# engcang/FAST-LIO-SAM-QN

Measured on AMD Instinct MI355X. Metric: scan-pair registrations/sec on 100k-pt clouds, higher is better.
Workload: dtype f32 search / f64 accumulate

## Files before the change

### fast-lio-sam-qn_amd/csrc/qn_batch.inc

```

namespace {

template <class F> void lanes_launch(const void* tab, dim3 grid, hipStream_t s, uint32_t shmem) {
  hipLaunchKernelGGL(HIP_KERNEL_NAME(k_lanes<F>), grid, dim3(F::TB), shmem, s, (const LaneEntry<typename F::Args>*)tab);
}
template <class A> void lane_push(std::vector<LaneEntry<A>>& v, const A& a, uint32_t nbx) {
  LaneEntry<A> e; memset((void*)&e, 0, sizeof(e)); e.a = a; e.nbx = nbx; v.push_back(e);
}

struct LanePlan {
  qn_ctx* c; size_t off = 0; bool overflow = false; int flush_rc = QN_OK;
  struct Item { void (*fn)(const void*, dim3, hipStream_t, uint32_t); size_t off; dim3 grid; int family; uint32_t shmem; };
  std::vector<Item> items;
  explicit LanePlan(qn_ctx* c_) : c(c_) {}
  template <class F> void add(const std::vector<LaneEntry<typename F::Args>>& e, int family, uint32_t shmem = 0) {
    if (e.empty()) return;
    size_t a = (off + 255) & ~(size_t)255; const size_t bytes = sizeof(LaneEntry<typename F::Args>) * e.size();
    if (a + bytes > c->args_cap) {
      if (items.empty() || bytes > c->args_cap || flush_rc != QN_OK) { overflow = true; return; }
      flush_rc = run();
      if (flush_rc == QN_OK && hipStreamSynchronize(c->stream) != hipSuccess) { c->last_error = "batch: stream synchronisation failed while flushing the argument arena"; flush_rc = QN_ERR_HIP; }
      if (flush_rc != QN_OK) { overflow = true; return; }
      a = 0;
    }
    memcpy(c->args_h + a, e.data(), bytes);
    uint32_t gx = 0; for (const auto& x : e) gx = std::max(gx, x.nbx);
    gx = (gx + 7u) & ~7u;
    items.push_back(Item{&lanes_launch<F>, a, dim3(gx, (uint32_t)e.size()), family, shmem});
    off = a + bytes;
  }
  int run() {
    if (overflow) { if (flush_rc == QN_OK) c->last_error = "batch: argument arena too small for one launch's table"; return QN_ERR_HIP; }
    if (items.empty()) return QN_OK;
    HIPCHK(c, hipMemcpyAsync(c->args_d, c->args_h, off, hipMemcpyHostToDevice, c->stream));
    for (const Item& it : items) { c->prof_begin(it.family, (int)it.grid.y); it.fn(c->args_d + it.off, it.grid, c->stream, it.shmem); c->prof_end(); }
    c->batch_launches += items.size();
    items.clear(); off = 0;
    HIPCHK(c, hipGetLastError());
    return QN_OK;
  }
};

struct ScratchSwap {
  qn_ctx* c;
  static void sw(qn_ctx* c) {
    std::swap(c->scan_sums, c->scan_sums2); std::swap(c->fb_list, c->fb_list2); std::swap(c->big_list, c->big_list2); std::swap(c->fb_count2, c->fb_count2b);
    std::swap(c->knn_idx, c->knn_idx2); std::swap(c->bbox_acc, c->bbox_acc2); std::swap(c->scan_status, c->scan_status2); std::swap(c->staging, c->staging2); std::swap(c->pin_up, c->pin_up2);
  }
  explicit ScratchSwap(qn_ctx* c_) : c(c_) { sw(c); }
  ~ScratchSwap() { sw(c); }
};

struct LaneRun {
  qn_ctx* c = nullptr; uint32_t pair = 0; bool active = false;
  int alias = -1;
  int ticks_left = 0, chunk = 0, chunk_start = 0, next = 0; bool first_chunk = true; long budget = 0;
  bool build_source = true;
};

int lane_set_cloud(qn_ctx* c, int which, const float* xyz, uint32_t n, uint32_t stride, bool on_device, hipStream_t s, GridLaunch* out) {
  CloudBuf& b = c->cloud[which];
  b.n = 0; b.has_grid = b.has_cov = false;
  if (n == 0) return QN_ERR_EMPTY_CLOUD;
  if (!xyz || stride < 12 || (stride & 3)) return QN_ERR_INVALID_ARG;
  if (n > c->max_points) return QN_ERR_CAPACITY;
  const char* dsrc = (const char*)xyz;
  if (!on_device) { const int rc = upload_host_cloud(c, xyz, n, stride, s, &dsrc); if (rc != QN_OK) return rc; }
  b.n = n;
  *out = prep_grid(c, b, dsrc, stride, true);
  return QN_OK;
}

bool batch_supported(const qn_ctx* c) {
  const qn_gicp_params& p = c->params;
  const int maxit = p.force_iterations > 0 ? p.force_iterations : p.max_iterations;
  return c->batch_lanes >= 2 && !c->lanes_failed && maxit > 0 && c->fused_ticks && c->fused_final && c->far_enabled && c->knn_hist && !c->verify_track && !c->clk_probe && !c->list_probe &&
         c->tick_tb == 512 && c->tick_occ >= 4 && !c->dbg_counters;
}

int batch_ensure_lanes(qn_ctx* c) {
  HIPCHK(c, hipSetDevice(c->device));
  const int B = std::max(1, std::min(c->batch_lanes, 64));
  if (c->lanes.empty()) c->lanes.push_back(c);
  while ((int)c->lanes.size() < B) {
    qn_ctx* l = nullptr;
    const int rc = (c->fail_lane_create > 0 && (int)c->lanes.size() >= c->fail_lane_create) ? QN_ERR_HIP : ctx_create(c->device, c->max_points, c->stream, &l);
    if (rc != QN_OK) {
      c->last_error = "batch: lane context creation failed (lanes need batch_lanes x the context's device memory)";
      while (c->lanes.size() > 1) { qn_ctx_destroy(c->lanes.back()); c->lanes.pop_back(); }
      (void)hipGetLastError();
      c->lanes_failed = true;
      return rc;
    }
    c->lanes.push_back(l);
  }
  if (!c->args_h) {
    c->args_cap = (size_t)4 << 20;
    HIPCHK(c, hipHostMalloc(&c->args_h, c->args_cap, hipHostMallocDefault));
    HIPCHK(c, hipMalloc(&c->args_d, c->args_cap));
  }
  for (qn_ctx* l : c->lanes) {
    if (l == c) continue;
    if (l->params.k_correspondences != c->params.k_correspondences) l->cloud[0].has_cov = l->cloud[1].has_cov = false;
    l->params = c->params;
    l->cell_override = c->cell_override; l->margin_nn = c->margin_nn; l->margin_nn_t0 = c->margin_nn_t0; l->margin_knn = c->margin_knn; l->big_blocks0 = c->big_blocks0; l->fb_blocks0 = c->fb_blocks0;
    l->big_ratio = c->big_ratio; l->nn_rounds = c->nn_rounds; l->knn_rounds = c->knn_rounds; l->knn_trips = c->knn_trips; l->knn_mm = c->knn_mm; l->knn_single_all = c->knn_single_all; l->bbox_blocks = c->bbox_blocks; l->stable_cells = c->stable_cells;
    l->unseeded_cap = c->unseeded_cap; l->track_from_tick = c->track_from_tick; l->fused_from_tick = c->fused_from_tick; l->ticks_per_chunk = c->ticks_per_chunk; l->far_chunk = c->far_chunk; l->far_group = c->far_group; l->far_ranked = c->far_ranked;
    l->list_small = c->list_small; l->tick_ppt_min = c->tick_ppt_min; l->tick_rpb = c->tick_rpb; l->nn_lane = c->nn_lane;
  }
  return QN_OK;
}

int batch_register(qn_ctx* owner, const qn_pair_desc* pairs, const uint32_t* idx, uint32_t m, double thr, qn_gicp_result* results, int* valid, int* status,
                   std::vector<const float*>& last_src, std::vector<uint64_t>& last_key) {
  hipStream_t s = owner->stream;
  const auto t_call = std::chrono::steady_clock::now();
  const qn_gicp_params& p = owner->params;
  const int k = p.k_correspondences;
  LanePlan plan(owner);
  std::vector<LaneRun> L(m);
  struct AliasGuard {
    std::vector<LaneRun>& L; std::vector<CloudBuf> saved; std::vector<double*> saved_nrm; std::vector<const float*>& last_src;
    AliasGuard(std::vector<LaneRun>& L_, std::vector<const float*>& ls) : L(L_), saved(L_.size()), saved_nrm(L_.size(), nullptr), last_src(ls) {}
    void borrow(size_t l, qn_ctx* from) { qn_ctx* c = L[l].c; saved[l] = c->cloud[0]; saved_nrm[l] = c->nrm_s_sorted; c->cloud[0] = from->cloud[0]; c->nrm_s_sorted = from->nrm_s_sorted; }
    ~AliasGuard() { for (size_t l = 0; l < L.size(); l++) if (L[l].alias >= 0 && saved_nrm[l]) { qn_ctx* c = L[l].c; c->cloud[0] = saved[l]; c->nrm_s_sorted = saved_nrm[l]; c->cloud[0].has_grid = c->cloud[0].has_cov = false; c->cloud[0].n = 0; last_src[l] = nullptr; } }
  } alias_guard(L, last_src);
  struct FailGuard { std::vector<LaneRun>& L; int* status; bool armed = true; ~FailGuard() { if (armed) for (const LaneRun& R : L) if (R.active) status[R.pair] = QN_ERR_HIP; } } fail_guard{L, status};
  std::vector<LaneEntry<PackBBoxK::Args>> v_pack; std::vector<LaneEntry<CellCountK::Args>> v_count; std::vector<LaneEntry<ScanLookbackK::Args>> v_scan;
  std::vector<LaneEntry<ScatterK::Args>> v_scat; std::vector<LaneEntry<StableCellsK::Args>> v_stab;
  std::vector<LaneEntry<KnnHistArgs>> v_sel, v_lst; std::vector<LaneEntry<KnnSingleK::Args>> v_single; std::vector<LaneEntry<KnnCovArgs>> v_tail; std::vector<LaneEntry<CovFromIdxK::Args>> v_cov;
  auto push_grid = [&](const GridLaunch& G) {
    lane_push(v_pack, G.pack, G.pack_nb); lane_push(v_count, G.count, G.nb); lane_push(v_scan, G.scan, G.scan_nb); lane_push(v_scat, G.scat, G.nb);
    if (G.stable) lane_push(v_stab, G.stab, G.nb);
  };
  auto push_knn = [&](const KnnLaunch& K) {
    lane_push(v_sel, K.sel, K.sel_nb); lane_push(v_lst, K.lst, K.lst_nb); lane_push(v_single, K.single, K.single_nb); lane_push(v_tail, K.tail, K.tail_nb); lane_push(v_cov, K.cov, K.cov_nb);
  };
  for (uint32_t l = 0; l < m; l++) {
    LaneRun& R = L[l]; R.c = owner->lanes[l]; R.pair = idx[l];
    qn_ctx* c = R.c;
    const qn_pair_desc& pd = pairs[R.pair];
    qn_gicp_result* out = &results[R.pair];
    valid[R.pair] = 0; memset(out, 0, sizeof(*out)); out->fitness = DBL_MAX;
    for (int i = 0; i < 4; i++) { out->T[5 * i] = 1.f; out->T64[5 * i] = 1.0; }
    c->pair_pipeline = false; c->persist_batch_off = true; c->tgt_pending = false; c->tgt_on_stream2 = false;
    const uint64_t key = ((uint64_t)pd.ns << 32) ^ ((uint64_t)pd.stride_bytes << 1) ^ (uint64_t)(pd.on_device ? 1 : 0);
    R.build_source = !(owner->batch_share_source && last_src[l] == pd.src && last_key[l] == key && pd.src != nullptr && c->cloud[0].has_grid && c->cloud[0].has_cov && c->cloud[0].n == pd.ns);
    if (R.build_source && owner->batch_share_source && pd.src != nullptr && pd.ns > 0) {
      for (uint32_t j = 0; j < l; j++) {
        const qn_pair_desc& pj = pairs[L[j].pair];
        if (L[j].active && L[j].alias < 0 && pj.src == pd.src && pj.ns == pd.ns && pj.stride_bytes == pd.stride_bytes && pj.on_device == pd.on_device) { R.alias = (int)j; break; }
      }
      if (R.alias >= 0) { alias_guard.borrow(l, L[R.alias].c); R.build_source = false; }
    }
    int rc = QN_OK; GridLaunch gs, gt;
    if (R.build_source) { last_src[l] = nullptr; rc = lane_set_cloud(c, QN_SOURCE, pd.src, pd.ns, pd.stride_bytes, pd.on_device != 0, s, &gs); }
    if (rc == QN_OK) { ScratchSwap sw(c); rc = lane_set_cloud(c, QN_TARGET, pd.dst, pd.nt, pd.stride_bytes, pd.on_device != 0, s, &gt); }
    if (rc == QN_ERR_HIP) return rc;
    status[R.pair] = rc;
    if (rc != QN_OK) {
      if (R.build_source) { c->cloud[0].has_grid = c->cloud[0].has_cov = false; c->cloud[0].n = 0; }
      c->cloud[1].has_grid = c->cloud[1].has_cov = false; c->cloud[1].n = 0;
      continue;
    }
    if (R.build_source) { push_grid(gs); push_knn(prep_knn(c, c->cloud[0], k, c->knn_idx, nullptr, true)); c->cloud[0].has_cov = true; }
    { ScratchSwap sw(c); push_grid(gt); push_knn(prep_knn(c, c->cloud[1], k, c->knn_idx, nullptr, true)); c->cloud[1].has_cov = true; }
    last_src[l] = R.alias >= 0 ? nullptr : pd.src; last_key[l] = key;
    R.active = true;
  }
  plan.add<PackBBoxK>(v_pack, QN_K_GRID_BUILD); plan.add<CellCountK>(v_count, QN_K_GRID_BUILD); plan.add<ScanLookbackK>(v_scan, QN_K_GRID_BUILD); plan.add<ScatterK>(v_scat, QN_K_GRID_BUILD); plan.add<StableCellsK>(v_stab, QN_K_GRID_BUILD);
  if (k <= 24) { if (owner->knn_mm) plan.add<KnnHistK<false, 32>>(v_sel, QN_K_KNN_SELECT, (uint32_t)owner->knn_lds_pad); else plan.add<KnnHistK<false, 32, false>>(v_sel, QN_K_KNN_SELECT, (uint32_t)owner->knn_lds_pad); plan.add<KnnHistK<true, 32>>(v_lst, QN_K_KNN_COV); } else { plan.add<KnnHistK<false, 48>>(v_sel, QN_K_KNN_SELECT); plan.add<KnnHistK<true, 48>>(v_lst, QN_K_KNN_COV); }
  plan.add<KnnSingleK>(v_single, QN_K_KNN_COV);
  if (k <= 16) plan.add<KnnCovK<16, true, 4>>(v_tail, QN_K_KNN_COV); else if (k <= 20) plan.add<KnnCovK<20, true, 4>>(v_tail, QN_K_KNN_COV); else if (k <= 24) plan.add<KnnCovK<24, true, 4>>(v_tail, QN_K_KNN_COV); else plan.add<KnnCovK<32, true, 4>>(v_tail, QN_K_KNN_COV);
  plan.add<CovFromIdxK>(v_cov, QN_K_KNN_COV);

  const int per_outer = p.optimizer == QN_OPT_LM ? 2 : 1;
  const int maxit = p.force_iterations > 0 ? p.force_iterations : p.max_iterations;
  const int fixed_unseeded = std::max(1, std::min(owner->track_from_tick, owner->fused_from_tick)) * per_outer;
  const bool exact_ticks = p.force_iterations > 0 && p.optimizer == QN_OPT_GN;
  {
    std::vector<LaneEntry<InitStateK::Args>> v_init;
    for (LaneRun& R : L) {
      if (!R.active) continue;
      qn_ctx* c = R.c;
      c->gen = 0; c->part_rows = 0; c->far_mode = 2; c->clear_far_now = true; c->unseeded_until = fixed_unseeded; c->count_far_now = false;
      c->result_host->phase = 0;
      R.ticks_left = exact_ticks ? maxit : 1 << 30;
      R.chunk = std::min(fixed_unseeded, R.ticks_left); R.chunk_start = 0; R.next = R.chunk; R.first_chunk = true;
      R.budget = (long)maxit * (p.optimizer == QN_OPT_LM ? (p.lm_max_iterations + 1) : 1) + 2;
      lane_push(v_init, InitStateK::Args{st_cur(c), c->guess_tmp, 0, 0, c->far_stats}, 1u);
    }
    plan.add<InitStateK>(v_init, QN_K_SOLVE);
  }
  auto finish_lane = [&](LaneRun& R, int rc) {
    qn_ctx* c = R.c;
    R.active = false;
    status[R.pair] = rc;
    if (rc != QN_OK) return;
    results[R.pair] = c->result_host->r;
    c->trace_len = c->result_host->trace_len; c->aligned_valid = true;
    valid[R.pair] = (results[R.pair].converged && results[R.pair].fitness < thr) ? 1 : 0;
  };
  struct ProfFlush { qn_ctx* c; ~ProfFlush() { c->prof_collect(); } } prof_flush{owner};
  int tick_no = 0;
  for (;;) {
    int stop = 1 << 30; bool any = false;
    for (const LaneRun& R : L) if (R.active) { any = true; stop = std::min(stop, R.next); }
    if (!any) break;
    for (; tick_no < stop; tick_no++) {
      {
        std::vector<LaneEntry<NnSearchArgs>> v_g, v_l; std::vector<LaneEntry<AccumulateK::Args>> v_acc;
        bool group = true, lane = true;
        for (LaneRun& R : L) {
          if (!R.active || tick_no >= R.c->unseeded_until) continue;
          qn_ctx* c = R.c;
          const int t = tick_no - R.chunk_start;
          c->count_far_now = R.first_chunk && (t / per_outer == (R.chunk - 1) / per_outer);
          const NnLaunch N = prep_nn(c, 0, c->sqd, false, tick_no / per_outer, 0);
          group = group && N.group; lane = lane && N.lane;
          lane_push(v_g, N.grid, N.grid_nb); lane_push(v_l, N.list, N.list_nb);
          const uint32_t nb = acc_blocks(c);
          lane_push(v_acc, prep_accumulate(c, 0, true), nb);
          c->count_far_now = false;
        }
        if (lane) plan.add<NnLaneK<0>>(v_g, QN_K_NN_SEARCH); else plan.add<NnSearchK<0, false, QN_NN_BLOCK>>(v_g, QN_K_NN_SEARCH);
        if (group) plan.add<NnSearchK<0, true, QN_BLOCK, true>>(v_l, QN_K_NN_FALLBACK); else plan.add<NnSearchK<0, true, QN_BLOCK>>(v_l, QN_K_NN_FALLBACK);
        plan.add<AccumulateK>(v_acc, QN_K_ACCUMULATE);
      }
      {
        std::vector<LaneEntry<TickArgs>> v_t; std::vector<LaneEntry<FarArgs>> v_f; std::vector<LaneEntry<FarReduceK::Args>> v_r;
        for (LaneRun& R : L) {
          if (!R.active || tick_no < R.c->unseeded_until) continue;
          qn_ctx* c = R.c;
          const TickArgs a = tick_args(c);
          lane_push(v_t, a, tick_blocks(c));
          if (a.far_mode == 1) { lane_push(v_f, far_args(c), (uint32_t)QN_FAR_BLOCKS); lane_push(v_r, far_reduce_args(c), 1u); }
          c->gen++; c->part_rows = -1;
        }
        plan.add<TickK<512, 4, 0, false>>(v_t, QN_K_GN_TICK_FUSED, (uint32_t)owner->tick_lds_pad); plan.add<FarK>(v_f, QN_K_FAR); plan.add<FarReduceK>(v_r, QN_K_FAR);
      }
    }
    {
      std::vector<LaneEntry<FinalizeK::Args>> v_fin; std::vector<LaneEntry<TickArgs>> v_close; std::vector<LaneEntry<FinalizeFitK::Args>> v_fit;
      for (LaneRun& R : L) {
        if (!R.active || R.next != stop) continue;
        qn_ctx* c = R.c;
        if (exact_ticks && R.ticks_left > R.chunk) lane_push(v_fin, FinalizeK::Args{st_cur(c), c->result_host, c->far_stats}, 1u);
        else {
          const TickArgs a = tick_args(c, 1);
          const uint32_t nb = tick_blocks(c);
          lane_push(v_close, a, nb);
          lane_push(v_fit, FinalizeFitK::Args{st_cur(c), c->result_host, c->far_stats, c->fit_psum, c->fit_pcnt, (int)tick_rows(c)}, 1u);
        }
// ... 68 lines not shown
```

### fast-lio-sam-qn_amd/csrc/qn_context.h

```cpp
#pragma once
#include <hip/hip_runtime.h>
#include <string>
#include <vector>
#include "qn_gicp_kernels.cuh"

struct CloudBuf {
  uint32_t n = 0, ncells = 0;
  bool has_grid = false, has_cov = false;
  float4* raw = nullptr;
  float4* sorted = nullptr;
  float4* sorted_tmp = nullptr;
  uint32_t* cell_of_pt = nullptr;
  uint32_t* cell_start = nullptr;
  uint32_t* counts = nullptr;
  double* nrm = nullptr;
  qn::GridView grid{};
  qn::GridDims* dims = nullptr;
  qn::GridDims* dims_host = nullptr;
};

struct ProfSpan { int family; hipEvent_t a, b; int count; };

struct qn_ctx {
  int device = 0;
  uint32_t max_points = 0, max_cells = 0;
  hipStream_t stream = nullptr; bool owns_stream = true;
  std::vector<qn_ctx*> lanes; int batch_lanes = 8; char* args_h = nullptr; char* args_d = nullptr; size_t args_cap = 0; uint64_t batch_launches = 0, batch_pairs = 0; bool is_lane = false, batch_trace = false, batch_share_source = true;
  bool lanes_failed = false; int fail_lane_create = 0;
  void* slab = nullptr;
  qn_gicp_params params{};
  CloudBuf cloud[2];
  qn::BBoxAcc* bbox_acc = nullptr; qn::BBoxAcc* bbox_acc2 = nullptr;
  unsigned long long* scan_status = nullptr; unsigned long long* scan_status2 = nullptr; uint32_t build_epoch = 0;
  int far_group = -1;
  int far_chunk = 2;
  bool batch_look = false;
  bool far_ranked = true;
  unsigned long long* list_probe = nullptr;
  bool device_look = true;
  bool clear_far_now = false;
  char* staging2 = nullptr;
  struct PinZone { char* h = nullptr; hipEvent_t ev = nullptr; bool busy = false; } pin_up, pin_up2;
  char* staging = nullptr;
  uint32_t* scan_sums = nullptr;

  qn::GicpState* state = nullptr;
  uint32_t gen = 0; int part_rows = 0;
  double* partials = nullptr;
  uint32_t* tail_ticket = nullptr;
  double* fit_psum = nullptr; uint32_t* fit_pcnt = nullptr;
  qn_iter_trace* trace = nullptr; uint32_t trace_len = 0;
  int32_t* corr = nullptr; int32_t* nn_idx = nullptr; int32_t* knn_idx = nullptr; float4* nn_ref = nullptr; double* nrm_s_sorted = nullptr; qn::TargetRec* tgt_rec = nullptr; float* sqd = nullptr; float* sqd_fit = nullptr;
  int32_t* far_cand = nullptr; float4* far_cand_ref = nullptr; float2* far_cand_b = nullptr; unsigned long long* far_req = nullptr; uint32_t* far_stats = nullptr; double* far_rows = nullptr; int far_mode = 2; bool far_enabled = true;
  uint2* fb_list = nullptr; uint2* big_list = nullptr; uint32_t* fb_count2 = nullptr;
  float4* aligned = nullptr; bool aligned_valid = false;
  double* pose_tmp = nullptr; float* guess_tmp = nullptr;
  qn::ResultBlock* result_host = nullptr; double* scalar_host = nullptr;
  int32_t* dbg_knn_idx = nullptr; float* dbg_knn_d2 = nullptr;
  qn_quatro_params qparams{}; bool qparams_set = false, q_ready = false; double q_last_scale = 1.0;
  float4* q_normals[2] = {nullptr, nullptr}; float* q_spfh[2] = {nullptr, nullptr}; float* q_fpfh_s[2] = {nullptr, nullptr}; float* q_fpfh[2] = {nullptr, nullptr};
  unsigned long long* q_key[2] = {nullptr, nullptr};
  float* q_pair[2] = {nullptr, nullptr}; uint32_t* q_pair_hash[2] = {nullptr, nullptr};
  uint32_t* q_hit = nullptr; uint32_t* q_list = nullptr; uint32_t* q_sel = nullptr; uint2* q_pairs = nullptr; uint32_t* q_counts = nullptr; double* q_T = nullptr;
  void* q_mm_c = nullptr; void* q_mm_q = nullptr; float* q_mm_qn = nullptr; uint32_t* q_mm_L = nullptr; unsigned long long* q_mm_table = nullptr; unsigned long long* q_mm_table_q = nullptr; bool feat_query_dedupe = false;
  uint32_t q_mm_mask = 0;
  uint2* q_mm_pairs = nullptr; uint32_t* q_mm_cnt = nullptr; uint32_t q_mm_cap = 0, q_mm_ncnt = 0; bool feat_mfma = true, feat_mm_retry = false; int feat_sample = 4 ; bool feat_verify = false; int feat_min_blocks = 1536; double q_wall_ms[3] = {0, 0, 0}; unsigned long long* q_mm_vkeys = nullptr; uint32_t* q_mm_vcnt = nullptr; uint32_t feat_fallbacks = 0, feat_survivors = 0;
  bool c2f_overlap = false;
  bool c2f_lanes_fpfh = false;
  bool tgt_early = true;
  bool quatro_fused = true;
  int normals_fg = 0, fpfh_fg = 0;
  float4* c2f_src = nullptr; float4* c2f_dst = nullptr;
  float* q_mean = nullptr; double* q_mean_psum = nullptr; void* q_host = nullptr;
  double cell_override = 0.0;
  int list_small = 6000;
  float big_ratio = 2.5f;
  bool fused_ticks = true;
  int nn_rounds = 1;
  int nn_lane = -1;
  int track_from_tick = 3;
  int fused_from_tick = 3;
  int unseeded_until = 3; bool count_far_now = false; int last_extra_unseeded = 0;
  int unseeded_cap = 10;
  int single_from_tick = 2;
  bool fused_final = true;
  int knn_rounds = 2;
  int knn_mm = 1;
  int knn_trips = 3;
  int knn_hist = 1;
  int big_blocks0 = 4096, fb_blocks0 = 512;
  float margin_nn_t0 = 0.f;
  float margin_nn = 1.f, margin_knn = 0.f;
  int margin_nn_cap = 3, margin_knn_cap = 5, ticks_per_chunk = 8; bool knn_single_all = false, stable_cells = true; int bbox_blocks = 64;
  hipStream_t stream2 = nullptr; hipEvent_t ev_pair = nullptr; bool pair_pipeline = true, pair_failed = false, tgt_on_stream2 = false, tgt_pending = false, no_pipe = false;
  uint32_t* scan_sums2 = nullptr; uint2* fb_list2 = nullptr; uint2* big_list2 = nullptr; uint32_t* fb_count2b = nullptr; int32_t* knn_idx2 = nullptr;
  uint32_t tick_ppt_min = 1;
  uint32_t tick_rpb = 2;
  uint32_t tick_tb = 512;
  int batch_min_share = 4;
  int knn_lds_pad = 0;
  int tick_lds_pad = 0;
  int tick_occ = 4;
  unsigned long long* pg_rows = nullptr; unsigned long long* pg_bc = nullptr; unsigned long long* pg_fit = nullptr; uint32_t* pg_status = nullptr; uint32_t* pg_status_host = nullptr;
  unsigned long long* pg_clk = nullptr; uint32_t pg_epoch = 0; bool prof_persist = false, persist = true, persist_batch_off = false, persist_fits = true; int persist_resident_blocks = 0; uint32_t persist_launches = 0, persist_gave_up = 0; unsigned long long persist_timeout = 25000000ull;
  uint32_t* dbg_counters = nullptr;
  unsigned long long* clk_probe = nullptr; uint32_t clk_n = 0;
  bool verify_track = false; int32_t* v_corr = nullptr; int32_t* v_nn_idx = nullptr; float* v_sqd = nullptr; float4* v_nn_ref = nullptr; uint32_t* v_counters = nullptr;
  bool prof_on = false, prof_open = false; int prof_depth = 0;
  std::vector<ProfSpan> spans;
  qn_kernel_stat stats[QN_K_COUNT] = {};
  std::string last_error;

  void set_error(const char* what, hipError_t e, int line);
  void prof_begin(int family, int count = 1); void prof_end(); void prof_collect();
};
```

### fast-lio-sam-qn_amd/csrc/qn_device.cuh

```cuda
#pragma once
#include <hip/hip_runtime.h>
#include <stdint.h>

namespace qn {

#define QN_TX 8
#define QN_TY 4
#define QN_TZ 4
#define QN_TILE_CELLS 128

struct GridDims {
  float ox, oy, oz, cell, inv_cell, eps;
  int nx, ny, nz, ntx, nty, ntz;
  uint32_t n;
  uint32_t ncells, nonfinite, pad;
};
struct GridView {
  const float4* pts;
  const uint32_t* cell_start;
  uint32_t* dbg;
  float ox, oy, oz, cell, inv_cell, eps;
  int nx, ny, nz;
  int ntx, nty, ntz;
  uint32_t n;
  const GridDims* dims;
};
__device__ __forceinline__ int uni(int v) { return __builtin_amdgcn_readfirstlane(v); }
__device__ __forceinline__ uint32_t uni(uint32_t v) { return (uint32_t)__builtin_amdgcn_readfirstlane((int)v); }
__device__ __forceinline__ float uni(float v) { return __int_as_float(__builtin_amdgcn_readfirstlane(__float_as_int(v))); }
__device__ __forceinline__ double uni(double v) { union { double d; int i[2]; } u; u.d = v; u.i[0] = __builtin_amdgcn_readfirstlane(u.i[0]); u.i[1] = __builtin_amdgcn_readfirstlane(u.i[1]); return u.d; }
__device__ __forceinline__ GridView grid_resolve(GridView g) {
  const GridDims d = *g.dims;
  g.ox = uni(d.ox); g.oy = uni(d.oy); g.oz = uni(d.oz); g.cell = uni(d.cell); g.inv_cell = uni(d.inv_cell); g.eps = uni(d.eps);
  g.nx = uni(d.nx); g.ny = uni(d.ny); g.nz = uni(d.nz); g.ntx = uni(d.ntx); g.nty = uni(d.nty); g.ntz = uni(d.ntz); g.n = uni(d.n);
  return g;
}

template <class A> struct alignas(16) LaneEntry { A a; uint32_t nbx; uint32_t pad_[3]; };
template <class F>
__global__ void __launch_bounds__(F::TB, F::OCC) k_lanes(const LaneEntry<typename F::Args>* __restrict__ tab) {
  const LaneEntry<typename F::Args>* e = tab + blockIdx.y;
  const uint32_t nbx = e->nbx;
  if (blockIdx.x >= nbx) return;
  F::run(e->a, blockIdx.x, nbx);
}

#define QN_INF_KEY 0xFFFFFFFFFFFFFFFFull

__device__ __forceinline__ int clampi(int v, int lo, int hi) { return v < lo ? lo : (v > hi ? hi : v); }
__device__ __forceinline__ int cell_coord(float v, float o, float inv, int n) {
  return clampi((int)floorf((v - o) * inv), 0, n - 1);
}
__device__ __forceinline__ uint32_t cell_key(const GridView& g, int x, int y, int z) {
  const uint32_t tile = ((uint32_t)(z >> 2) * g.nty + (y >> 2)) * g.ntx + (x >> 3);
  return (tile << 7) | ((z & 3) << 5) | ((y & 3) << 3) | (x & 7);
}
__device__ __forceinline__ unsigned long long pack_key(float d2, uint32_t idx) {
  return ((unsigned long long)__float_as_uint(d2) << 32) | idx;
}
__device__ __forceinline__ float key_d2(unsigned long long k) { return __uint_as_float((uint32_t)(k >> 32)); }
__device__ __forceinline__ uint32_t key_idx(unsigned long long k) { return (uint32_t)k; }

typedef float qn_f2 __attribute__((ext_vector_type(2)));
__device__ __forceinline__ float sqdist(float qx, float qy, float qz, float px, float py, float pz) {
  const qn_f2 q = {qx, qy}, p = {px, py};
  const qn_f2 d = q - p;
  const qn_f2 d2 = d * d;
  const float dz = qz - pz;
  return (d2.x + d2.y) + dz * dz;
}

__device__ __forceinline__ int rfl(int v) { return __builtin_amdgcn_readfirstlane(v); }
__device__ __forceinline__ uint32_t rflu(uint32_t v) { return (uint32_t)__builtin_amdgcn_readfirstlane((int)v); }
__device__ __forceinline__ int rdlane(int v, int l) { return __builtin_amdgcn_readlane(v, l); }
__device__ __forceinline__ uint32_t rdlane(uint32_t v, int l) { return (uint32_t)__builtin_amdgcn_readlane((int)v, l); }
__device__ __forceinline__ float rdlane(float v, int l) { return __int_as_float(__builtin_amdgcn_readlane(__float_as_int(v), l)); }

#if defined(QN_INST_GROUP) && QN_INST_GROUP == 10
__device__ __forceinline__ int wave_min_i(int v) {
#pragma unroll
  for (int o = 32; o > 0; o >>= 1) { int t = __shfl_xor(v, o); v = t < v ? t : v; }
  return v;
}
__device__ __forceinline__ int wave_max_i(int v) {
#pragma unroll
  for (int o = 32; o > 0; o >>= 1) { int t = __shfl_xor(v, o); v = t > v ? t : v; }
  return v;
}
__device__ __forceinline__ unsigned long long wave_min_u64(unsigned long long v) {
#pragma unroll
  for (int o = 32; o > 0; o >>= 1) { unsigned long long t = __shfl_xor(v, o); v = t < v ? t : v; }
  return v;
}
__device__ __forceinline__ float wave_min_f(float v) {
#pragma unroll
  for (int o = 32; o > 0; o >>= 1) v = fminf(v, __shfl_xor(v, o));
  return v;
}
__device__ __forceinline__ float wave_max_f(float v) {
#pragma unroll
  for (int o = 32; o > 0; o >>= 1) v = fmaxf(v, __shfl_xor(v, o));
  return v;
}
// ... 166 lines not shown
  int k, cnt;
  __device__ __forceinline__ void reset() {
    w = QN_INF_KEY; cnt = 0;
    int kk = k; asm volatile("" : "+s"(kk));
#pragma unroll
    for (int j = 0; j < KMAX; j++) a[j] = (j < KMAX - kk) ? 0ull : QN_INF_KEY;
  }
  __device__ __forceinline__ void init(int k_, unsigned long long (*pend_)[64], uint32_t* dbg_ = nullptr) {
    k = k_; pend = pend_; dbg = dbg_; reset();
  }
  __device__ __forceinline__ bool slot_valid(int j) const { return j >= KMAX - k && a[j] != QN_INF_KEY; }
  __device__ __forceinline__ void refresh() { w = a[KMAX - 1]; }
  __device__ __forceinline__ void insert(unsigned long long key) {
#pragma unroll
    for (int j = 0; j < KMAX; j++) {
      unsigned long long lo = key < a[j] ? key : a[j];
      unsigned long long hi = key < a[j] ? a[j] : key;
      a[j] = lo; key = hi;
    }
  }
  __device__ __forceinline__ void flush() {
    const int lane = threadIdx.x & 63;
    const int m = wave_max_i(cnt);
    for (int e = 0; e < m; e++) {
      unsigned long long key = e < cnt ? pend[e][lane] : QN_INF_KEY;
      insert(key);
    }
    cnt = 0;
    refresh();
    if (dbg && lane == 0) atomicAdd(&dbg[2], 1u);
  }
  __device__ __forceinline__ void consider(bool on, float d2, uint32_t idx) {
    const unsigned long long key = pack_key(d2, idx);
    if (on && key < w) { pend[cnt][threadIdx.x & 63] = key; cnt++; }
    if (__any(cnt == QN_PEND_CAP)) flush();
  }
  __device__ __forceinline__ void merge_from(int lane_xor, bool recv) {
    if (KMAX > 24) {
      unsigned long long tmp[KMAX];
#pragma unroll
      for (int j = 0; j < KMAX; j++) tmp[j] = __shfl_xor(a[j], lane_xor);
#pragma unroll 1
      for (int j = 0; j < KMAX; j++) {
        unsigned long long other = QN_INF_KEY;
#pragma unroll
        for (int u = 0; u < KMAX; u++) other = (u == j) ? tmp[u] : other;
        if (__any(j >= KMAX - k)) insert((recv && j >= KMAX - k) ? other : QN_INF_KEY);
      }
      return;
    }
#pragma unroll
    for (int j = 0; j < KMAX; j++) {
      const unsigned long long other = __shfl_xor(a[j], lane_xor);
      if (__any(j >= KMAX - k)) insert((recv && j >= KMAX - k) ? other : QN_INF_KEY);
    }
  }
  template <int S>
  __device__ __forceinline__ void finish(bool on) {
    if (__any(cnt > 0)) flush();
    if (S == 1) return;
    const int lane = threadIdx.x & 63;
    merge_from(32, on && (lane & 32) == 0);
    if (S == 4) merge_from(16, on && (lane & 48) == 0);
    refresh();
    const unsigned long long w0 = __shfl(w, lane & (64 / S - 1));
    if (on) w = w0;
  }
  __device__ __forceinline__ bool full() const { return w != QN_INF_KEY; }
  __device__ __forceinline__ float worst_d2() const { return key_d2(w); }
  __device__ __forceinline__ int found() const {
    int f = 0;
#pragma unroll
    for (int j = 0; j < KMAX; j++) f += (j >= KMAX - k && a[j] != QN_INF_KEY) ? 1 : 0;
    return f;
  }
  __device__ __forceinline__ int wanted() const { return k; }
};

__device__ __forceinline__ float tile_box_d2(const GridView& g, int tx, int ty, int tz, float qx, float qy, float qz) {
  const float xl = g.ox + (float)(tx << 3) * g.cell, xh = g.ox + (float)min((tx << 3) + 8, g.nx) * g.cell;
  const float yl = g.oy + (float)(ty << 2) * g.cell, yh = g.oy + (float)min((ty << 2) + 4, g.ny) * g.cell;
  const float zl = g.oz + (float)(tz << 2) * g.cell, zh = g.oz + (float)min((tz << 2) + 4, g.nz) * g.cell;
  const float dx = fmaxf(fmaxf(xl - qx, qx - xh) - g.eps, 0.f), dy = fmaxf(fmaxf(yl - qy, qy - yh) - g.eps, 0.f), dz = fmaxf(fmaxf(zl - qz, qz - zh) - g.eps, 0.f);
  return ((dx * dx + dy * dy) + dz * dz) * 0.999998f;
}

__device__ __forceinline__ void divmod_small(int n, int d, int& q, int& r) {
  q = (int)((float)n * __builtin_amdgcn_rcpf((float)d));
  r = n - q * d;
  if (r < 0) { q--; r += d; }
  if (r >= d) { q++; r -= d; }
}

template <class Body>
__device__ __forceinline__ uint32_t stream_box(const GridView& g, int x0, int x1, int y0, int y1, int z0, int z1, const bool tile_mode, WaveLds* lds, Body&& body,
                                               const float bqx = 0.f, const float bqy = 0.f, const float bqz = 0.f, const float ball_r2 = -1.f) {
  const int lane = threadIdx.x & 63;
  const int tx0 = x0 >> 3, ntr = (x1 >> 3) - tx0 + 1, nyr = y1 - y0 + 1;
  const int ty0 = y0 >> 2, ntyr = (y1 >> 2) - ty0 + 1;
  const int nseg = tile_mode ? ntr * ntyr * ((z1 >> 2) - (z0 >> 2) + 1) : ntr * nyr * (z1 - z0 + 1);
  uint32_t grand = 0;
  for (int sb = 0; sb < nseg; sb += 64) {
    const int sidx = sb + lane;
    uint32_t s = 0, len = 0;
    if (sidx < nseg) {
      int t, r; divmod_small(sidx, ntr, r, t);
      if (tile_mode) {
        int qz_, ry_; divmod_small(r, ntyr, qz_, ry_);
        const int tzz = (z0 >> 2) + qz_, tyy = ty0 + ry_, txx = tx0 + t;
        const uint32_t tile = ((uint32_t)tzz * g.nty + tyy) * g.ntx + txx;
        if (!(ball_r2 >= 0.f && tile_box_d2(g, txx, tyy, tzz, bqx, bqy, bqz) > ball_r2)) { s = g.cell_start[tile << 7]; len = g.cell_start[(tile + 1) << 7] - s; }
      } else {
        int qz_, ry_; divmod_small(r, nyr, qz_, ry_);
        const int ry = y0 + ry_, rz = z0 + qz_, tx = tx0 + t;
        const int xa = max(x0, tx << 3), xb = min(x1, (tx << 3) + 7);
        const uint32_t k0 = cell_key(g, xa, ry, rz);
        s = g.cell_start[k0]; len = g.cell_start[k0 + (xb - xa) + 1] - s;
      }
    }
    const uint32_t incl = wave_incl_scan_u32(len, lane);
    const uint32_t total = rdlane(incl, 63);
    if (total == 0) continue;
    wave_lds_fence();
    lds->seg_excl[lane] = incl - len; lds->seg_start[lane] = s;
    wave_lds_fence();
    for (uint32_t cb = 0; cb < total; cb += 64) {
      const uint32_t slot = cb + lane;
      const bool valid = slot < total;
      const int j = chunk_segment(lds->tile_cid, cb, incl - len, incl);
      float4 p = make_float4(0.f, 0.f, 0.f, 0.f);
      if (valid) p = g.pts[lds->seg_start[j] + (slot - lds->seg_excl[j])];
      body(p, valid, min(64u, total - cb));
    }
    grand += total;
  }
  return grand;
}

#define QN_CL_DX 8
#define QN_CL_DY 4
#define QN_CL_DZ 4

template <int S>
__device__ __forceinline__ void build_clusters(const GridView& g, WaveLds* lds, unsigned long long todo, int cx, int cy, int cz,
                                               float qx, float qy, float qz, float r, uint32_t& cid, int& ncl, uint32_t& nseg_all) {
  const int lane = threadIdx.x & 63;
  const bool mine = (todo >> lane) & 1ull;
  cid = 0xffffffffu; ncl = 0;
  for (unsigned long long rem = todo; rem != 0; ncl++) {
    const int leader = __ffsll((long long)rem) - 1;
    const int ax = rdlane(cx, leader), ay = rdlane(cy, leader), az = rdlane(cz, leader);
    const bool in = ((rem >> lane) & 1ull) && abs(cx - ax) <= QN_CL_DX && abs(cy - ay) <= QN_CL_DY && abs(cz - az) <= QN_CL_DZ;
    if (in) cid = ncl;
    rem &= ~__ballot(in);
  }
  wave_lds_fence();
  if (lane < ncl) { lds->box[lane][0] = 0x3fffffff; lds->box[lane][1] = -1; lds->box[lane][2] = 0x3fffffff; lds->box[lane][3] = -1; lds->box[lane][4] = 0x3fffffff; lds->box[lane][5] = -1; }
  wave_lds_fence();
  if (mine && lane < 64 / S) {
    atomicMin(&lds->box[cid][0], cell_coord(qx - r, g.ox, g.inv_cell, g.nx)); atomicMax(&lds->box[cid][1], cell_coord(qx + r, g.ox, g.inv_cell, g.nx));
    atomicMin(&lds->box[cid][2], cell_coord(qy - r, g.oy, g.inv_cell, g.ny)); atomicMax(&lds->box[cid][3], cell_coord(qy + r, g.oy, g.inv_cell, g.ny));
    atomicMin(&lds->box[cid][4], cell_coord(qz - r, g.oz, g.inv_cell, g.nz)); atomicMax(&lds->box[cid][5], cell_coord(qz + r, g.oz, g.inv_cell, g.nz));
  }
  wave_lds_fence();
  uint32_t my_nseg = 0;
  if (lane < ncl) {
    int* b = lds->box[lane];
    my_nseg = (uint32_t)(((b[1] >> 3) - (b[0] >> 3) + 1) * (b[3] - b[2] + 1) * (b[5] - b[4] + 1));
    uint32_t tm = 0;
    if (my_nseg > 384) {
      tm = 1;
      b[0] = (b[0] >> 3) << 3; b[1] = min(((b[1] >> 3) << 3) + 7, g.nx - 1);
      b[2] = (b[2] >> 2) << 2; b[3] = min(((b[3] >> 2) << 2) + 3, g.ny - 1);
      b[4] = (b[4] >> 2) << 2; b[5] = min(((b[5] >> 2) << 2) + 3, g.nz - 1);
      my_nseg = (uint32_t)(((b[1] >> 3) - (b[0] >> 3) + 1) * ((b[3] >> 2) - (b[2] >> 2) + 1) * ((b[5] >> 2) - (b[4] >> 2) + 1));
    }
    lds->cl_tile_mode[lane] = tm;
  }
  const uint32_t seg_incl = wave_incl_scan_u32(my_nseg, lane);
  nseg_all = rdlane(seg_incl, 63);
  lds->cl_seg0[lane] = seg_incl - my_nseg;
  if (lane == 0) lds->cl_seg0[64] = nseg_all;
  wave_lds_fence();
}

template <int S, class Fn>
__device__ __forceinline__ void stream_chunks(const GridView& g, WaveLds* lds, const uint32_t total, Fn&& fn) {
  const int lane = threadIdx.x & 63;
  const float INF = __int_as_float(0x7f800000);
  const uint32_t ex = lds->seg_excl[lane], nxs = lane < 63 ? lds->seg_excl[(lane + 1) & 63] : total;
  for (uint32_t cb = 0; cb < total; cb += 64) {
    const uint32_t slot = cb + lane;
    const int j = chunk_segment(lds->tile_cid, cb, ex, nxs);
    const uint32_t cnt = min(64u, total - cb);
// ... 80 lines not shown
    bool retry = false;
    if (mine) {
      const int* b = lds->box[cid];
      const int ex0 = b[0], ex1 = b[1], ey0 = b[2], ey1 = b[3], ez0 = b[4], ez1 = b[5];
      const float INF = __int_as_float(0x7f800000);
      float d = INF;
      if (ex0 > 0) d = fminf(d, qx - (g.ox + ex0 * g.cell));
      if (ex1 < g.nx - 1) d = fminf(d, (g.ox + (ex1 + 1) * g.cell) - qx);
      if (ey0 > 0) d = fminf(d, qy - (g.oy + ey0 * g.cell));
      if (ey1 < g.ny - 1) d = fminf(d, (g.oy + (ey1 + 1) * g.cell) - qy);
      if (ez0 > 0) d = fminf(d, qz - (g.oz + ez0 * g.cell));
      if (ez1 < g.nz - 1) d = fminf(d, (g.oz + (ez1 + 1) * g.cell) - qz);
      if (d == INF || !(r == r)) { certified = true; d_unseen = INF; }
      else { d -= g.eps; d_unseen = d; certified = d > 0.f && sink.full() && sink.worst_d2() < d * d; }
      if (!certified) {
        if (sink.full()) r = fmaxf(sqrtf(sink.worst_d2()) * 1.000001f + g.eps, r + g.eps);
        else {
          const int f = sink.found();
          r = f > 0 ? fmaxf(r * sqrtf((float)sink.wanted() / (float)f) * 1.25f, r + g.cell) : 2.f * r + g.cell;
        }
        r = fminf(r, r_cap);
        if (round + 1 < max_rounds) { retry = true; sink.reset(); }
      }
    }
    todo = __ballot(retry);
    if (g.dbg && lane == 0 && todo) atomicAdd(&g.dbg[3], (uint32_t)__popcll(todo));
  }
  return certified;
}

struct CapBox {
  float o2[3];
  float S;
};
__device__ __forceinline__ CapBox cap_of(const GridView& g, float qx, float qy, float qz) {
  CapBox c;
  const float ox = fmaxf(fmaxf(g.ox - qx, qx - (g.ox + g.nx * g.cell)), 0.f);
  const float oy = fmaxf(fmaxf(g.oy - qy, qy - (g.oy + g.ny * g.cell)), 0.f);
  const float oz = fmaxf(fmaxf(g.oz - qz, qz - (g.oz + g.nz * g.cell)), 0.f);
  c.o2[0] = ox * ox; c.o2[1] = oy * oy; c.o2[2] = oz * oz; c.S = (c.o2[0] + c.o2[1]) + c.o2[2];
  return c;
}
__device__ __forceinline__ float cap_extent(const GridView& g, const CapBox& c, float r, int axis) {
  const float rest = c.S - c.o2[axis];
  if (rest <= 0.f) return r;
  const float v = r * r - rest * 0.999999f;
  return v > 0.f ? sqrtf(v) * 1.000001f + g.eps : g.eps;
}
__device__ __forceinline__ float cap_face_dist(const CapBox& c, float f, int axis) {
  const float rest = (c.S - c.o2[axis]) * 0.999999f;
  return rest > 0.f ? sqrtf(f * f + rest) * 0.999999f : f;
}

struct SingleStats { uint32_t rounds, cand, segs; float r_first, r_last; };
__device__ __forceinline__ void wave_search_single(const GridView& g, float qx, float qy, float qz, float r, const float r_cap,
                                                   unsigned long long& best_out, float& second_out, float& d_unseen, WaveLds* lds, SingleStats& st_out, const bool stats) {
  const int lane = threadIdx.x & 63;
  const float INF = __int_as_float(0x7f800000);
  const CapBox cap = cap_of(g, qx, qy, qz);
  if (cap.S > 0.f) r = fminf(fmaxf(r, sqrtf(cap.S) + g.cell), fmaxf(r_cap, r));
  if (stats) { st_out.rounds = 0; st_out.cand = 0; st_out.segs = 0; st_out.r_first = r; }
  float done2 = -1.f;
  int ptx0 = 0, ptx1 = -1, pty0 = 0, pty1 = -1, ptz0 = 0, ptz1 = -1;
  unsigned long long best = QN_INF_KEY; float second = INF;
  for (int round = 0;; round++) {
    const float rx = cap_extent(g, cap, r, 0), ry = cap_extent(g, cap, r, 1), rz = cap_extent(g, cap, r, 2);
    int x0 = rfl(cell_coord(qx - rx, g.ox, g.inv_cell, g.nx)), x1 = rfl(cell_coord(qx + rx, g.ox, g.inv_cell, g.nx));
    int y0 = rfl(cell_coord(qy - ry, g.oy, g.inv_cell, g.ny)), y1 = rfl(cell_coord(qy + ry, g.oy, g.inv_cell, g.ny));
    int z0 = rfl(cell_coord(qz - rz, g.oz, g.inv_cell, g.nz)), z1 = rfl(cell_coord(qz + rz, g.oz, g.inv_cell, g.nz));
    const int tx0 = x0 >> 3, ntr = (x1 >> 3) - tx0 + 1;
    int nseg = ntr * (y1 - y0 + 1) * (z1 - z0 + 1);
    const bool tile_mode = nseg > 128;
    int ty0 = 0, ntyr = 1;
    if (tile_mode) {
      x0 = (x0 >> 3) << 3; x1 = min(((x1 >> 3) << 3) + 7, g.nx - 1);
      y0 = (y0 >> 2) << 2; y1 = min(((y1 >> 2) << 2) + 3, g.ny - 1);
      z0 = (z0 >> 2) << 2; z1 = min(((z1 >> 2) << 2) + 3, g.nz - 1);
      ty0 = y0 >> 2; ntyr = (y1 >> 2) - ty0 + 1;
      nseg = ntr * ntyr * ((z1 >> 2) - (z0 >> 2) + 1);
    }
    const int nyr = y1 - y0 + 1;
    if (!tile_mode || done2 < 0.f) { best = QN_INF_KEY; second = INF; done2 = -1.f; }
    const float in2 = r * r * 1.000002f;
    for (int sb = 0; sb < nseg; sb += 64) {
      const int sidx = sb + lane;
      uint32_t s = 0, len = 0;
      if (sidx < nseg) {
        int t, rr; divmod_small(sidx, ntr, rr, t);
        if (tile_mode) {
          int qz_, ry_; divmod_small(rr, ntyr, qz_, ry_);
          const int tzz = (z0 >> 2) + qz_, tyy = ty0 + ry_, txx = tx0 + t;
          const uint32_t tile = ((uint32_t)tzz * g.nty + tyy) * g.ntx + txx;
          const float tb2 = tile_box_d2(g, txx, tyy, tzz, qx, qy, qz);
          const bool seen = tb2 <= done2 && txx >= ptx0 && txx <= ptx1 && tyy >= pty0 && tyy <= pty1 && tzz >= ptz0 && tzz <= ptz1;
          if (!(tb2 > in2) && !seen) { s = g.cell_start[tile << 7]; len = g.cell_start[(tile + 1) << 7] - s; }
        } else {
          int qz_, ry_; divmod_small(rr, nyr, qz_, ry_);
          const int ry = y0 + ry_, rz = z0 + qz_, tx = tx0 + t;
          const int xa = max(x0, tx << 3), xb = min(x1, (tx << 3) + 7);
          const uint32_t k0 = cell_key(g, xa, ry, rz);
          s = g.cell_start[k0]; len = g.cell_start[k0 + (xb - xa) + 1] - s;
        }
      }
      const uint32_t incl = wave_incl_scan_u32(len, lane);
      const uint32_t total = rdlane(incl, 63);
      if (total == 0) continue;
      if (g.dbg && lane == 0) atomicAdd(&g.dbg[11], total);
      if (stats) st_out.cand += total;
      wave_lds_fence();
      lds->seg_excl[lane] = incl - len; lds->seg_start[lane] = s;
      wave_lds_fence();
      for (uint32_t cb = 0; cb < total; cb += 64) {
        const uint32_t slot = cb + lane;
        const int j = chunk_segment(lds->tile_cid, cb, incl - len, incl);
        if (slot < total) {
          const float4 p = g.pts[lds->seg_start[j] + (slot - lds->seg_excl[j])];
          const float d2 = sqdist(qx, qy, qz, p.x, p.y, p.z);
          const unsigned long long k = pack_key(d2, __float_as_uint(p.w));
          if (k < best) { if (best != QN_INF_KEY) second = key_d2(best); best = k; }
          else if (d2 < second) second = d2;
        }
      }
    }
    if (g.dbg && lane == 0) { atomicAdd(&g.dbg[10], 1u); atomicAdd(&g.dbg[12], (uint32_t)nseg); if (round == 0) atomicAdd(&g.dbg[13], 1u); }
    if (stats) { st_out.rounds++; st_out.segs += (uint32_t)nseg; st_out.r_last = r; }
    if (tile_mode) { done2 = in2; ptx0 = tx0; ptx1 = tx0 + ntr - 1; pty0 = ty0; pty1 = ty0 + ntyr - 1; ptz0 = z0 >> 2; ptz1 = z1 >> 2; }
    const unsigned long long b = wave_min_u64(best);
    float c = (best == b) ? second : key_d2(best);
    if (best == QN_INF_KEY) c = INF;
    c = wave_min_f(c);
    float d = INF;
    if (x0 > 0) d = fminf(d, cap_face_dist(cap, qx - (g.ox + x0 * g.cell), 0));
    if (x1 < g.nx - 1) d = fminf(d, cap_face_dist(cap, (g.ox + (x1 + 1) * g.cell) - qx, 0));
    if (y0 > 0) d = fminf(d, cap_face_dist(cap, qy - (g.oy + y0 * g.cell), 1));
    if (y1 < g.ny - 1) d = fminf(d, cap_face_dist(cap, (g.oy + (y1 + 1) * g.cell) - qy, 1));
    if (z0 > 0) d = fminf(d, cap_face_dist(cap, qz - (g.oz + z0 * g.cell), 2));
    if (z1 < g.nz - 1) d = fminf(d, cap_face_dist(cap, (g.oz + (z1 + 1) * g.cell) - qz, 2));
    bool cert;
    if (tile_mode && r == r && round <= 160) d = fminf(d, r * 0.999998f + g.eps);
    if (d == INF || !(r == r) || round > 160) { cert = true; d_unseen = INF; }
    else { d -= g.eps; d_unseen = d; cert = d > 0.f && b != QN_INF_KEY && key_d2(b) < d * d; }
    if (cert) { best_out = b; second_out = c; return; }
    r = (b != QN_INF_KEY) ? fmaxf(sqrtf(key_d2(b)) * 1.000001f + g.eps, r + g.eps) : (r > 6.f * g.cell ? r + (2.f + round) * g.cell : 2.f * r + g.cell);
    r = fminf(r, r_cap);
  }
}

__device__ __forceinline__ void wave_search_single(const GridView& g, float qx, float qy, float qz, float r, const float r_cap,
                                                   unsigned long long& best_out, float& second_out, float& d_unseen, WaveLds* lds) {
  SingleStats none;
  wave_search_single(g, qx, qy, qz, r, r_cap, best_out, second_out, d_unseen, lds, none, false);
}

__device__ __forceinline__ void wave_search_far16(const GridView& g, float qx_in, float qy_in, float qz_in, bool member_in, float r_in,
                                                  unsigned long long& best_out, float& second_out, float& d_unseen_out, WaveLds* lds) {
  const int lane = threadIdx.x & 63;
  const float INF = __int_as_float(0x7f800000);
  const unsigned long long mm = __ballot(member_in) & 0xffffull;
  const int m = __popcll(mm);
  int m2 = 1; while (m2 < m) m2 <<= 1;
  const int S = 64 / m2;
  const int my_rank = __popcll(mm & ((1ull << (lane & 15)) - 1ull));
  wave_lds_fence();
  if (member_in && lane < 16) lds->seg_cid[my_rank] = (uint32_t)lane;
  wave_lds_fence();
  const int rk = lane & (m2 - 1);
  const bool has_q = rk < m;
  const int src_lane = has_q ? (int)lds->seg_cid[rk] : 0;
  const float qx = __shfl(qx_in, src_lane), qy = __shfl(qy_in, src_lane), qz = __shfl(qz_in, src_lane), r = __shfl(r_in, src_lane);
  const uint32_t sub = (uint32_t)(lane / m2);
  const float cqx = 0.5f * (wave_min_f(has_q ? qx : INF) + wave_max_f(has_q ? qx : -INF));
  const float cqy = 0.5f * (wave_min_f(has_q ? qy : INF) + wave_max_f(has_q ? qy : -INF));
  const float cqz = 0.5f * (wave_min_f(has_q ? qz : INF) + wave_max_f(has_q ? qz : -INF));
  const float off = has_q ? sqrtf(sqdist(qx, qy, qz, cqx, cqy, cqz)) * 1.000002f + 1e-30f : 0.f;
  float R = wave_max_f(has_q ? r + off : 0.f);
  const CapBox cap = cap_of(g, cqx, cqy, cqz);
  if (cap.S > 0.f) R = fmaxf(R, sqrtf(cap.S) + g.cell);
  Best1 sink; sink.init();
  bool open = has_q;
  unsigned long long fin_b = QN_INF_KEY; float fin_s = INF, fin_d = INF;
  float done2 = -1.f; int ptx0 = 0, ptx1 = -1, pty0 = 0, pty1 = -1, ptz0 = 0, ptz1 = -1;
  for (int round = 0;; round++) {
    const float rx = cap_extent(g, cap, R, 0), ry = cap_extent(g, cap, R, 1), rz = cap_extent(g, cap, R, 2);
    int x0 = rfl(cell_coord(cqx - rx, g.ox, g.inv_cell, g.nx)), x1 = rfl(cell_coord(cqx + rx, g.ox, g.inv_cell, g.nx));
    int y0 = rfl(cell_coord(cqy - ry, g.oy, g.inv_cell, g.ny)), y1 = rfl(cell_coord(cqy + ry, g.oy, g.inv_cell, g.ny));
    int z0 = rfl(cell_coord(cqz - rz, g.oz, g.inv_cell, g.nz)), z1 = rfl(cell_coord(cqz + rz, g.oz, g.inv_cell, g.nz));
    x0 = (x0 >> 3) << 3; x1 = min(((x1 >> 3) << 3) + 7, g.nx - 1);
    y0 = (y0 >> 2) << 2; y1 = min(((y1 >> 2) << 2) + 3, g.ny - 1);
    z0 = (z0 >> 2) << 2; z1 = min(((z1 >> 2) << 2) + 3, g.nz - 1);
    const int tx0 = x0 >> 3, ntr = (x1 >> 3) - tx0 + 1, ty0 = y0 >> 2, ntyr = (y1 >> 2) - ty0 + 1, tz0 = z0 >> 2;
    const int nseg = ntr * ntyr * ((z1 >> 2) - tz0 + 1);
    const float in2 = R * R * 1.000002f;
    bool left_out = false;
    for (int sb = 0; sb < nseg; sb += 64) {
      const int sidx = sb + lane;
      uint32_t s = 0, len = 0;
      if (sidx < nseg) {
        int t, rr; divmod_small(sidx, ntr, rr, t);
        int qz_, ry_; divmod_small(rr, ntyr, qz_, ry_);
        const int tzz = tz0 + qz_, tyy = ty0 + ry_, txx = tx0 + t;
        const uint32_t tile = ((uint32_t)tzz * g.nty + tyy) * g.ntx + txx;
        const float tb2 = tile_box_d2(g, txx, tyy, tzz, cqx, cqy, cqz);
        const bool seen = tb2 <= done2 && txx >= ptx0 && txx <= ptx1 && tyy >= pty0 && tyy <= pty1 && tzz >= ptz0 && tzz <= ptz1;
        if (tb2 > in2) left_out = true;
        else if (!seen) { s = g.cell_start[tile << 7]; len = g.cell_start[(tile + 1) << 7] - s; }
      }
      const uint32_t incl = wave_incl_scan_u32(len, lane);
      const uint32_t total = rdlane(incl, 63);
      if (total == 0) continue;
      if (g.dbg && lane == 0) atomicAdd(&g.dbg[11], total);
      wave_lds_fence();
      lds->seg_excl[lane] = incl - len; lds->seg_start[lane] = s;
      wave_lds_fence();
      for (uint32_t cb = 0; cb < total; cb += 64) {
        const uint32_t slot = cb + lane;
        const int j = chunk_segment(lds->tile_cid, cb, incl - len, incl);
        const uint32_t cnt = min(64u, total - cb);
        wave_lds_fence();
        if (slot < total) lds->tile[lane] = g.pts[lds->seg_start[j] + (slot - lds->seg_excl[j])];
        wave_lds_fence();
        for (uint32_t c = 0; c < cnt; c += 4u * (uint32_t)S) {
          float4 cp[4]; uint32_t ci[4];
#pragma unroll
          for (int u = 0; u < 4; u++) { ci[u] = c + (uint32_t)(u * S) + sub; cp[u] = lds->tile[ci[u] & 63u]; }
#pragma unroll
          for (int u = 0; u < 4; u++) sink.consider(open && ci[u] < cnt, sqdist(qx, qy, qz, cp[u].x, cp[u].y, cp[u].z), __float_as_uint(cp[u].w));
        }
      }
    }
    if (g.dbg && lane == 0) { atomicAdd(&g.dbg[10], 1u); atomicAdd(&g.dbg[12], (uint32_t)nseg); if (round == 0) atomicAdd(&g.dbg[13], 1u); }
    done2 = in2; ptx0 = tx0; ptx1 = tx0 + ntr - 1; pty0 = ty0; pty1 = ty0 + ntyr - 1; ptz0 = tz0; ptz1 = z1 >> 2;
    const bool everything = !__any(left_out) && x0 == 0 && x1 == g.nx - 1 && y0 == 0 && y1 == g.ny - 1 && z0 == 0 && z1 == g.nz - 1;
    unsigned long long b = sink.key;
    for (int o = m2; o < 64; o <<= 1) { const unsigned long long t = __shfl_xor(b, o); b = t < b ? t : b; }
    float sc = (sink.key == b) ? sink.second : key_d2(sink.key);
    if (sink.key == QN_INF_KEY) sc = INF;
    for (int o = m2; o < 64; o <<= 1) sc = fminf(sc, __shfl_xor(sc, o));
    float need = 0.f;
    if (open) {
      const float d = R * 0.999998f - off - g.eps;
      bool cert;
      if (everything || round > 160 || !(R == R)) { cert = true; fin_d = INF; }
      else { cert = d > 0.f && b != QN_INF_KEY && key_d2(b) < d * d; fin_d = fmaxf(d, 0.f); }
      if (cert) { fin_b = b; fin_s = sc; open = false; }
      else if (b != QN_INF_KEY) need = sqrtf(key_d2(b)) * 1.000002f + 2.f * g.eps + off;
    }
    if (!__any(open)) break;
    const float want = wave_max_f(need);
    const float grown = want > 0.f ? want : (R > 6.f * g.cell ? R + (2.f + round) * g.cell : 2.f * R + g.cell);
    R = fmaxf(grown, R * 1.0001f + g.eps);
  }
  const unsigned long long ob = __shfl(fin_b, my_rank & 63); const float os = __shfl(fin_s, my_rank & 63), od = __shfl(fin_d, my_rank & 63);
  if (member_in) { best_out = ob; second_out = os; d_unseen_out = od; }
}

template <int KMAX>
__device__ __forceinline__ void lane_ball_knn(const GridView& g, float qx, float qy, float qz, float r, BestK<KMAX>& sink) {
  for (int round = 0;; round++) {
    sink.reset();
    const int bx0 = cell_coord(qx - r, g.ox, g.inv_cell, g.nx), bx1 = cell_coord(qx + r, g.ox, g.inv_cell, g.nx);
    const int by0 = cell_coord(qy - r, g.oy, g.inv_cell, g.ny), by1 = cell_coord(qy + r, g.oy, g.inv_cell, g.ny);
    const int bz0 = cell_coord(qz - r, g.oz, g.inv_cell, g.nz), bz1 = cell_coord(qz + r, g.oz, g.inv_cell, g.nz);
    const bool all = bx0 == 0 && by0 == 0 && bz0 == 0 && bx1 == g.nx - 1 && by1 == g.ny - 1 && bz1 == g.nz - 1;
    for (int rz = bz0; rz <= bz1; rz++) for (int ry = by0; ry <= by1; ry++) for (int tx = bx0 >> 3; tx <= (bx1 >> 3); tx++) {
      const int xa = max(bx0, tx << 3), xb = min(bx1, (tx << 3) + 7);
      const uint32_t k0 = cell_key(g, xa, ry, rz);
      const uint32_t s = g.cell_start[k0], e = g.cell_start[k0 + (xb - xa) + 1];
      for (uint32_t i = s; i < e; i++) {
        const float4 p = g.pts[i];
        const unsigned long long key = pack_key(sqdist(qx, qy, qz, p.x, p.y, p.z), __float_as_uint(p.w));
        if (key < sink.w) { sink.insert(key); sink.refresh(); }
      }
    }
    if (all || round > 160) return;
    if (sink.full()) {
      const float bd = sqrtf(sink.worst_d2()) * 1.000001f + g.eps;
      if (bd <= r) return;
      r = bd;
    } else {
      r = 2.f * r + g.cell;
    }
  }
}

struct M3 { double m[3][3]; };

__device__ __forceinline__ M3 m3_inverse(const M3& a) {
  const double (*m)[3] = a.m;
  double c00 = m[1][1]*m[2][2] - m[1][2]*m[2][1];
  double c01 = m[1][2]*m[2][0] - m[1][0]*m[2][2];
  double c02 = m[1][0]*m[2][1] - m[1][1]*m[2][0];
  double det = m[0][0]*c00 + m[0][1]*c01 + m[0][2]*c02;
  double id = 1.0 / det;
  M3 r;
  r.m[0][0] = c00*id; r.m[1][0] = c01*id; r.m[2][0] = c02*id;
  r.m[0][1] = (m[0][2]*m[2][1] - m[0][1]*m[2][2])*id;
  r.m[1][1] = (m[0][0]*m[2][2] - m[0][2]*m[2][0])*id;
  r.m[2][1] = (m[0][1]*m[2][0] - m[0][0]*m[2][1])*id;
  r.m[0][2] = (m[0][1]*m[1][2] - m[0][2]*m[1][1])*id;
  r.m[1][2] = (m[0][2]*m[1][0] - m[0][0]*m[1][2])*id;
  r.m[2][2] = (m[0][0]*m[1][1] - m[0][1]*m[1][0])*id;
  return r;
}

__device__ inline void sym_eig3(const double A[6] , double w[3], double V[3][3]) {
  double a[3][3] = {{A[0], A[1], A[2]}, {A[1], A[3], A[4]}, {A[2], A[4], A[5]}};
  double v[3][3] = {{1, 0, 0}, {0, 1, 0}, {0, 0, 1}};
  for (int sweep = 0; sweep < 32; sweep++) {
    double off = fabs(a[0][1]) + fabs(a[0][2]) + fabs(a[1][2]);
    double diag = fabs(a[0][0]) + fabs(a[1][1]) + fabs(a[2][2]);
    if (off <= 1e-300 || off <= 1e-17 * diag) break;
#pragma unroll
    for (int pq = 0; pq < 3; pq++) {
      const int p = pq == 2 ? 1 : 0, q = pq == 0 ? 1 : 2;
      if (a[p][q] == 0.0) continue;
      double theta = (a[q][q] - a[p][p]) / (2.0 * a[p][q]);
      double t = (theta >= 0 ? 1.0 : -1.0) / (fabs(theta) + sqrt(theta * theta + 1.0));
      double c = 1.0 / sqrt(t * t + 1.0), s = t * c;
#pragma unroll
      for (int k = 0; k < 3; k++) { double akp = a[k][p], akq = a[k][q]; a[k][p] = c*akp - s*akq; a[k][q] = s*akp + c*akq; }
#pragma unroll
      for (int k = 0; k < 3; k++) { double apk = a[p][k], aqk = a[q][k]; a[p][k] = c*apk - s*aqk; a[q][k] = s*apk + c*aqk; }
#pragma unroll
      for (int k = 0; k < 3; k++) { double vkp = v[k][p], vkq = v[k][q]; v[k][p] = c*vkp - s*vkq; v[k][q] = s*vkp + c*vkq; }
    }
  }
  double e0 = a[0][0], e1 = a[1][1], e2 = a[2][2];
  int i0 = 0, i1 = 1, i2 = 2;
  if (e0 < e1) { double t = e0; e0 = e1; e1 = t; int ti = i0; i0 = i1; i1 = ti; }
  if (e1 < e2) { double t = e1; e1 = e2; e2 = t; int ti = i1; i1 = i2; i2 = ti; }
  if (e0 < e1) { double t = e0; e0 = e1; e1 = t; int ti = i0; i0 = i1; i1 = ti; }
  w[0] = e0; w[1] = e1; w[2] = e2;
// ... 10 lines not shown
```

### fast-lio-sam-qn_amd/csrc/qn_engine.hip

```cpp
#include <hip/hip_runtime.h>
#include <cfloat>
#include <cmath>
#include <cstdio>
#include <cstring>
#include <string>
#include <vector>
#include <atomic>
#include <thread>
#include <chrono>
#include "qn_instances.h"
#include "qn_context.h"
#include "qn_selftest.cuh"
#include "qn_pool.h"

using namespace qn;

#define HIPCHK(ctx, call)                                                                 \
  do { hipError_t e_ = (call);                                                            \
       if (e_ != hipSuccess) { (ctx)->set_error(#call, e_, __LINE__); return QN_ERR_HIP; } \
  } while (0)

void qn_ctx::set_error(const char* what, hipError_t e, int line) {
  char buf[512]; snprintf(buf, sizeof(buf), "%s -> %s (qn_engine.hip:%d)", what, hipGetErrorString(e), line);
  last_error = buf;
}

void qn_ctx::prof_begin(int family, int count) {
  if (!prof_on) return;
  if (prof_open) { prof_depth++; return; }
  ProfSpan sp; sp.family = family; sp.count = count;
  if (hipEventCreate(&sp.a) != hipSuccess) return;
  if (hipEventCreate(&sp.b) != hipSuccess) { hipEventDestroy(sp.a); return; }
  hipEventRecord(sp.a, stream);
  spans.push_back(sp);
  prof_open = true; prof_depth = 0;
}
void qn_ctx::prof_end() {
  if (!prof_on || spans.empty() || !prof_open) return;
  if (prof_depth > 0) { prof_depth--; return; }
  prof_open = false;
  hipEventRecord(spans.back().b, stream);
}
void qn_ctx::prof_collect() {
  for (auto& sp : spans) {
    float ms = 0; if (hipEventSynchronize(sp.b) == hipSuccess && hipEventElapsedTime(&ms, sp.a, sp.b) == hipSuccess) { stats[sp.family].total_ms += ms; stats[sp.family].launches += sp.count; }
    hipEventDestroy(sp.a); hipEventDestroy(sp.b);
  }
  spans.clear(); prof_open = false; prof_depth = 0;
}
struct ProfScope { qn_ctx* c; ProfScope(qn_ctx* c_, int fam) : c(c_) { c->prof_begin(fam); } ~ProfScope() { c->prof_end(); } };

extern "C" const char* qn_status_str(int s) {
  switch (s) {
    case QN_OK: return "ok"; case QN_ERR_INVALID_ARG: return "invalid argument"; case QN_ERR_EMPTY_CLOUD: return "empty cloud";
    case QN_ERR_CAPACITY: return "cloud exceeds context capacity"; case QN_ERR_NOT_READY: return "clouds/covariances not set";
    case QN_ERR_HIP: return "HIP runtime error"; case QN_ERR_NO_DEVICE: return "no gfx950 device (no CPU fallback)";
  }
  return "unknown status";
}
extern "C" const char* qn_last_error(const qn_ctx* ctx) { return ctx ? ctx->last_error.c_str() : "null context"; }

extern "C" void qn_gicp_default_params(qn_gicp_params* p) {
  if (!p) return;
  memset(p, 0, sizeof(*p));
  p->k_correspondences = 20; p->max_iterations = 64; p->max_corr_dist = (double)FLT_MAX;
  p->transformation_epsilon = 5e-4; p->rotation_epsilon = 2e-3; p->optimizer = QN_OPT_LM;
  p->lm_max_iterations = 10; p->lm_init_lambda_factor = 1e-9; p->force_iterations = 0;
  p->ransac_iterations = 0; p->ransac_outlier_threshold = 0.05; p->euclidean_fitness_epsilon = -DBL_MAX;
}

struct Slab {
  char* base = nullptr; size_t off = 0, cap = 0;
  template <class T> void take(T*& p, size_t bytes) {
    const size_t a = (off + 255) & ~(size_t)255;
    if (base) p = (T*)(base + a);
    off = a + bytes;
  }
};
static void carve_cloud(qn_ctx* c, Slab& sl, CloudBuf& b) {
  sl.take(b.raw, sizeof(float4) * c->max_points);
  sl.take(b.sorted, sizeof(float4) * c->max_points);
  sl.take(b.sorted_tmp, sizeof(float4) * c->max_points);
  sl.take(b.cell_of_pt, sizeof(uint32_t) * c->max_points);
  sl.take(b.cell_start, sizeof(uint32_t) * ((size_t)c->max_cells + 1));
  sl.take(b.counts, sizeof(uint32_t) * ((size_t)c->max_cells + 1));
  sl.take(b.nrm, sizeof(double) * 3 * c->max_points);
  sl.take(b.dims, sizeof(GridDims));
}

static int ctx_create(int device, uint32_t max_points, hipStream_t shared_stream, qn_ctx** out);
extern "C" int qn_ctx_create(int device, uint32_t max_points, qn_ctx** out) { return ctx_create(device, max_points, nullptr, out); }
static int ctx_create(int device, uint32_t max_points, hipStream_t shared_stream, qn_ctx** out) {
  if (!out || max_points == 0) return QN_ERR_INVALID_ARG;
  *out = nullptr;
  int ndev = 0;
  if (hipGetDeviceCount(&ndev) != hipSuccess || ndev <= 0 || device < 0 || device >= ndev) return QN_ERR_NO_DEVICE;
  qn_ctx* c = new qn_ctx();
  c->device = device; c->max_points = max_points;
  size_t mc = (size_t)max_points * 16; if (mc < (1u << 18)) mc = 1u << 18; if (mc > (1u << 23)) mc = 1u << 23;
  c->max_cells = (uint32_t)mc;
  qn_gicp_default_params(&c->params);
  int rc = QN_OK;
  auto fail = [&](int code) { qn_ctx_destroy(c); return code; };
  if (hipSetDevice(device) != hipSuccess) return fail(QN_ERR_NO_DEVICE);
  if (shared_stream) { c->stream = shared_stream; c->owns_stream = false; c->is_lane = true; }
  else if (hipStreamCreateWithFlags(&c->stream, hipStreamNonBlocking) != hipSuccess) return fail(QN_ERR_HIP);
#define CA(call) if ((call) != hipSuccess) return fail(QN_ERR_HIP)
  auto carve = [&](Slab& sl) {
    carve_cloud(c, sl, c->cloud[0]);
    carve_cloud(c, sl, c->cloud[1]);
    sl.take(c->staging, (size_t)max_points * 32);
    sl.take(c->scan_sums, sizeof(uint32_t) * (c->max_cells / (QN_BLOCK * QN_SCAN_ITEMS) + 2));
    sl.take(c->state, 2 * sizeof(GicpState));
    sl.take(c->partials, 2 * sizeof(double) * (QN_ACC_MAX_BLOCKS + 8) * QN_NPART);
    sl.take(c->nn_idx, sizeof(int32_t) * max_points);
    sl.take(c->knn_idx, sizeof(int32_t) * (size_t)max_points * 32);
    sl.take(c->nn_ref, sizeof(float4) * max_points);
    sl.take(c->nrm_s_sorted, sizeof(double) * 3 * max_points);
    sl.take(c->tgt_rec, sizeof(TargetRec) * max_points);
    sl.take(c->fit_psum, sizeof(double) * (QN_ACC_MAX_BLOCKS + 8));
    sl.take(c->fit_pcnt, sizeof(uint32_t) * (QN_ACC_MAX_BLOCKS + 8));
    sl.take(c->trace, sizeof(qn_iter_trace) * QN_MAX_TRACE);
    sl.take(c->corr, sizeof(int32_t) * max_points);
    sl.take(c->sqd, sizeof(float) * max_points);
    sl.take(c->sqd_fit, sizeof(float) * max_points);
    sl.take(c->far_cand, sizeof(int32_t) * QN_FAR_M * (size_t)max_points);
    sl.take(c->far_cand_ref, sizeof(float4) * max_points);
    sl.take(c->far_cand_b, sizeof(float2) * max_points);
    sl.take(c->far_req, sizeof(unsigned long long) * (max_points / 64 + 2));
    sl.take(c->far_stats, 4 * sizeof(uint32_t));
    sl.take(c->far_rows, sizeof(double) * QN_FAR_BLOCKS * QN_NPART);
    sl.take(c->fb_list, sizeof(uint2) * max_points);
    sl.take(c->big_list, sizeof(uint2) * max_points);
    sl.take(c->fb_count2, 4 * sizeof(uint32_t));
    sl.take(c->aligned, sizeof(float4) * max_points);
    sl.take(c->pose_tmp, sizeof(double) * 16);
    sl.take(c->guess_tmp, sizeof(float) * 16);
    sl.take(c->scan_sums2, sizeof(uint32_t) * (c->max_cells / (QN_BLOCK * QN_SCAN_ITEMS) + 2));
    sl.take(c->fb_list2, sizeof(uint2) * max_points);
    sl.take(c->big_list2, sizeof(uint2) * max_points);
    sl.take(c->fb_count2b, 4 * sizeof(uint32_t));
    sl.take(c->knn_idx2, sizeof(int32_t) * (size_t)max_points * 32);
    sl.take(c->staging2, (size_t)max_points * 32);
    sl.take(c->bbox_acc, 2 * (QN_BBOX_MAX_BLOCKS + 1) * sizeof(BBoxAcc)); c->bbox_acc2 = c->bbox_acc ? c->bbox_acc + (QN_BBOX_MAX_BLOCKS + 1) : nullptr;
    sl.take(c->scan_status, sizeof(unsigned long long) * 2 * (c->max_cells / (QN_BLOCK * QN_SCAN_ITEMS) + 2)); c->scan_status2 = c->scan_status ? c->scan_status + (c->max_cells / (QN_BLOCK * QN_SCAN_ITEMS) + 2) : nullptr;
    sl.take(c->pg_rows, sizeof(unsigned long long) * 3 * QN_PERSIST_ROWS * QN_PERSIST_RSTRIDE);
    sl.take(c->pg_bc, sizeof(unsigned long long) * 64);
    sl.take(c->pg_fit, sizeof(unsigned long long) * (QN_PERSIST_MAX_BLOCKS + 1) * 4);
    sl.take(c->pg_status, 4 * sizeof(uint32_t));
    sl.take(c->tail_ticket, 4 * sizeof(uint32_t));
  };
  { Slab dry; carve(dry);
    Slab sl; sl.cap = (dry.off + ((size_t)2 << 20) - 1) & ~(((size_t)2 << 20) - 1);
    CA(hipMalloc(&c->slab, sl.cap)); sl.base = (char*)c->slab; carve(sl); }
  CA(hipMemsetAsync(c->far_stats, 0, 4 * sizeof(uint32_t), c->stream));
  CA(hipHostMalloc(&c->result_host, sizeof(ResultBlock), hipHostMallocDefault));
  for (int w = 0; w < 2; w++) { CA(hipHostMalloc(&c->cloud[w].dims_host, sizeof(GridDims), hipHostMallocDefault)); memset(c->cloud[w].dims_host, 0, sizeof(GridDims)); }
  CA(hipHostMalloc(&c->scalar_host, 64 * sizeof(double), hipHostMallocDefault));
  CA(hipHostMalloc(&c->pg_status_host, 4 * sizeof(uint32_t), hipHostMallocDefault));
  CA(hipMemsetAsync(c->pg_rows, 0xFF, sizeof(unsigned long long) * 3 * QN_PERSIST_ROWS * QN_PERSIST_RSTRIDE, c->stream));
  CA(hipMemsetAsync(c->pg_bc, 0, sizeof(unsigned long long) * 64, c->stream));
  CA(hipMemsetAsync(c->pg_fit, 0, sizeof(unsigned long long) * (QN_PERSIST_MAX_BLOCKS + 1) * 4, c->stream));
  CA(hipMemsetAsync(c->pg_status, 0, 4 * sizeof(uint32_t), c->stream));
  CA(hipMemsetAsync(c->tail_ticket, 0, 4 * sizeof(uint32_t), c->stream));
  CA(hipMemsetAsync(c->state, 0, 2 * sizeof(GicpState), c->stream));
  hipLaunchKernelGGL(k_bbox_acc_init, dim3(1), dim3(256), 0, c->stream, c->bbox_acc, 2 * (QN_BBOX_MAX_BLOCKS + 1));
  CA(hipMemsetAsync(c->fb_count2, 0, 4 * sizeof(uint32_t), c->stream)); CA(hipMemsetAsync(c->fb_count2b, 0, 4 * sizeof(uint32_t), c->stream));
  CA(hipMemsetAsync(c->scan_status, 0, sizeof(unsigned long long) * 2 * (c->max_cells / (QN_BLOCK * QN_SCAN_ITEMS) + 2), c->stream));
  for (int w = 0; w < 2; w++) CA(hipMemsetAsync(c->cloud[w].counts, 0, sizeof(uint32_t) * ((size_t)c->max_cells + 1), c->stream));
  CA(hipMemsetAsync(c->knn_idx, 0xff, sizeof(int32_t) * (size_t)max_points * 32, c->stream));
// ... 18 lines not shown
  for (qn_ctx* l : c->lanes) if (l != c) qn_ctx_destroy(l);
  c->lanes.clear();
  if (c->args_h) hipHostFree(c->args_h);
  hipFree(c->args_d);
  c->prof_collect();
  hipFree(c->slab);
  hipFree(c->q_mm_c); hipFree(c->q_mm_q); hipFree(c->q_mm_qn); hipFree(c->q_mm_L); hipFree(c->q_mm_table); hipFree(c->q_mm_table_q); hipFree(c->q_mm_pairs); hipFree(c->q_mm_cnt); hipFree(c->q_mm_vkeys); hipFree(c->q_mm_vcnt);
  for (int w = 0; w < 2; w++) { hipFree(c->q_normals[w]); hipFree(c->q_spfh[w]); hipFree(c->q_fpfh_s[w]); hipFree(c->q_fpfh[w]); hipFree(c->q_key[w]); hipFree(c->q_pair[w]); hipFree(c->q_pair_hash[w]); }
  hipFree(c->q_hit); hipFree(c->q_list); hipFree(c->q_sel); hipFree(c->q_pairs); hipFree(c->q_counts); hipFree(c->q_T); hipFree(c->q_mean); hipFree(c->q_mean_psum);
  if (c->q_host) hipHostFree(c->q_host);
  hipFree(c->c2f_src); hipFree(c->c2f_dst);
  hipFree(c->dbg_knn_idx); hipFree(c->dbg_knn_d2); hipFree(c->dbg_counters);
  hipFree(c->v_corr); hipFree(c->v_nn_idx); hipFree(c->v_sqd); hipFree(c->v_nn_ref); hipFree(c->v_counters);
  if (c->result_host) hipHostFree(c->result_host);
  for (int w = 0; w < 2; w++) if (c->cloud[w].dims_host) hipHostFree(c->cloud[w].dims_host);
  if (c->scalar_host) hipHostFree(c->scalar_host);
  hipFree(c->pg_clk); if (c->list_probe) hipFree(c->list_probe); if (c->pg_status_host) hipHostFree(c->pg_status_host);
  if (c->ev_pair) hipEventDestroy(c->ev_pair);
  for (qn_ctx::PinZone* z : {&c->pin_up, &c->pin_up2}) { if (z->ev) hipEventDestroy(z->ev); if (z->h) hipHostFree(z->h); }
  if (c->stream2) { hipStreamSynchronize(c->stream2); hipStreamDestroy(c->stream2); }
  if (c->stream && c->owns_stream) hipStreamDestroy(c->stream);
  delete c;
}

static int clouds_valid(qn_ctx* c);
extern "C" void* qn_ctx_stream(qn_ctx* c) { return c ? (void*)c->stream : nullptr; }
extern "C" int qn_ctx_synchronize(qn_ctx* c) {
  if (!c) return QN_ERR_INVALID_ARG;
  HIPCHK(c, hipStreamSynchronize(c->stream));
  if (c->stream2) HIPCHK(c, hipStreamSynchronize(c->stream2));
  c->prof_collect();
  return clouds_valid(c);
}

extern "C" int qn_gicp_set_params(qn_ctx* c, const qn_gicp_params* p) {
  if (!c || !p) return QN_ERR_INVALID_ARG;
  if (p->k_correspondences < 1 || p->k_correspondences > 32 || p->max_iterations < 0 || p->lm_max_iterations < 1 ||
      (p->optimizer != QN_OPT_LM && p->optimizer != QN_OPT_GN) || !(p->max_corr_dist > 0)) return QN_ERR_INVALID_ARG;
  if (p->k_correspondences != c->params.k_correspondences) { c->cloud[0].has_cov = c->cloud[1].has_cov = false; }
  c->params = *p;
  return QN_OK;
}

extern "C" int qn_gicp_get_params(const qn_ctx* c, qn_gicp_params* p) { if (!c || !p) return QN_ERR_INVALID_ARG; *p = c->params; return QN_OK; }

static GicpConfig make_cfg(const qn_ctx* c) {
  GicpConfig g; const qn_gicp_params& p = c->params;
  g.k = p.k_correspondences; g.max_iterations = p.max_iterations; g.optimizer = p.optimizer; g.lm_max_iterations = p.lm_max_iterations;
  g.force_iterations = p.force_iterations; g.max_corr_dist_sq = p.max_corr_dist * p.max_corr_dist;
  g.transformation_epsilon = p.transformation_epsilon; g.rotation_epsilon = p.rotation_epsilon; g.lm_init_lambda_factor = p.lm_init_lambda_factor;
  return g;
}

static inline GicpState* st_cur(qn_ctx* c) { return c->state + (c->gen & 1u); }
static inline GicpState* st_nxt(qn_ctx* c) { return c->state + ((c->gen + 1u) & 1u); }
static inline double* part_cur(qn_ctx* c) { return c->partials + (size_t)(c->gen & 1u) * (QN_ACC_MAX_BLOCKS + 8) * QN_NPART; }
static inline double* part_nxt(qn_ctx* c) { return c->partials + (size_t)((c->gen + 1u) & 1u) * (QN_ACC_MAX_BLOCKS + 8) * QN_NPART; }

static bool pair_pipeline_ready(qn_ctx* c) {
  if (c->stream2) return true;
  if (c->pair_failed || !c->knn_idx2) return false;
  const bool ok = hipStreamCreateWithFlags(&c->stream2, hipStreamNonBlocking) == hipSuccess && hipEventCreateWithFlags(&c->ev_pair, hipEventDisableTiming) == hipSuccess;
  if (!ok) { c->pair_failed = true; if (c->stream2) { hipStreamDestroy(c->stream2); c->stream2 = nullptr; } (void)hipGetLastError(); }
  return ok;
}
static void swap_scratch(qn_ctx* c) {
  std::swap(c->stream, c->stream2); std::swap(c->scan_sums, c->scan_sums2); std::swap(c->fb_list, c->fb_list2); std::swap(c->big_list, c->big_list2);
  std::swap(c->fb_count2, c->fb_count2b); std::swap(c->knn_idx, c->knn_idx2);
  std::swap(c->bbox_acc, c->bbox_acc2); std::swap(c->scan_status, c->scan_status2);
  std::swap(c->pin_up, c->pin_up2);
  std::swap(c->staging, c->staging2);
}
struct TargetScope {
  qn_ctx* c; bool on;
  TargetScope(qn_ctx* c_, bool on_) : c(c_), on(on_) { if (on) swap_scratch(c); }
  ~TargetScope() { if (on) { (void)hipEventRecord(c->ev_pair, c->stream); swap_scratch(c); c->tgt_pending = true; } }
};
static int join_target(qn_ctx* c) {
  if (!c->tgt_pending) return QN_OK;
  c->tgt_pending = false;
  return hipStreamWaitEvent(c->stream, c->ev_pair, 0) == hipSuccess ? QN_OK : QN_ERR_HIP;
}

struct GridLaunch { PackBBoxK::Args pack; uint32_t pack_nb; CellCountK::Args count; ScanLookbackK::Args scan; uint32_t scan_nb; ScatterK::Args scat; StableCellsK::Args stab; bool stable; uint32_t nb; };
static GridLaunch prep_grid(qn_ctx* c, CloudBuf& b, const char* dsrc, uint32_t stride, bool lanes = false) {
  const uint32_t n = b.n;
  GridView& g = b.grid;
  memset(&g, 0, sizeof(g));
  g.pts = b.sorted; g.cell_start = b.cell_start; g.dbg = c->dbg_counters; g.n = n; g.dims = b.dims;
  GridLaunch L;
  L.nb = (n + QN_BLOCK - 1) / QN_BLOCK;
  L.scan_nb = (c->max_cells + QN_BLOCK * QN_SCAN_ITEMS - 1) / (QN_BLOCK * QN_SCAN_ITEMS);
  if (((++c->build_epoch) & 0x3fffffffu) == 0u) ++c->build_epoch;
  L.pack_nb = std::min<uint32_t>(L.nb, (uint32_t)std::min(lanes ? QN_BBOX_MAX_BLOCKS : c->bbox_blocks, QN_BBOX_MAX_BLOCKS));
  L.pack = PackBBoxK::Args{dsrc, stride, n, b.raw, c->bbox_acc, c->max_cells, c->cell_override, b.dims, b.dims_host};
  L.count = CellCountK::Args{b.raw, n, g, b.counts, b.cell_of_pt};
  L.scan = ScanLookbackK::Args{b.counts, b.dims, b.cell_start, c->scan_status, c->build_epoch, n};
  L.stable = c->stable_cells;
  L.scat = ScatterK::Args{b.raw, n, b.cell_of_pt, b.cell_start, b.counts, L.stable ? b.sorted_tmp : b.sorted};
  L.stab = StableCellsK::Args{b.sorted_tmp, n, b.cell_of_pt, b.cell_start, b.sorted};
  b.has_grid = true; b.has_cov = false;
  return L;
}
static int build_grid(qn_ctx* c, CloudBuf& b, const char* dsrc, uint32_t stride) {
  hipStream_t s = c->stream;
  const GridLaunch L = prep_grid(c, b, dsrc, stride);
  { ProfScope ps(c, QN_K_GRID_BUILD);
    hipLaunchKernelGGL(k_pack_bbox_dims, dim3(L.pack_nb), dim3(QN_BLOCK), 0, s, L.pack.in, L.pack.stride, L.pack.n, L.pack.raw, L.pack.acc, L.pack.max_cells, L.pack.cell_override, L.pack.dims_dev, L.pack.dims_host);
    hipLaunchKernelGGL(k_cell_count, dim3(L.nb), dim3(QN_BLOCK), 0, s, L.count.pts, L.count.n, L.count.g, L.count.counts, L.count.cell_of_pt);
    hipLaunchKernelGGL(k_scan_lookback, dim3(L.scan_nb), dim3(QN_BLOCK), 0, s, L.scan.in, L.scan.dims, L.scan.out, L.scan.status, L.scan.epoch, L.scan.total);
    hipLaunchKernelGGL(k_scatter, dim3(L.nb), dim3(QN_BLOCK), 0, s, L.scat.pts, L.scat.n, L.scat.cell_of_pt, L.scat.cell_start, L.scat.counts, L.scat.sorted);
    if (L.stable) hipLaunchKernelGGL(k_stable_cells, dim3(L.nb), dim3(QN_BLOCK), 0, s, L.stab.in, L.stab.n, L.stab.cell_of_pt, L.stab.cell_start, L.stab.out); }
  HIPCHK(c, hipGetLastError());
  return QN_OK;
}
static int clouds_valid(qn_ctx* c) {
  for (int w = 0; w < 2; w++)
    if (c->cloud[w].has_grid && c->cloud[w].dims_host && c->cloud[w].dims_host->nonfinite) {
      c->last_error = w == 0 ? "source cloud contains non-finite coordinates (is_dense == false clouds are not supported)" : "target cloud contains non-finite coordinates (is_dense == false clouds are not supported)";
      c->cloud[w].has_grid = c->cloud[w].has_cov = false;
      return QN_ERR_INVALID_ARG;
    }
  return QN_OK;
}

static int upload_host_cloud(qn_ctx* c, const float* xyz, uint32_t n, uint32_t& stride, hipStream_t s, const char** dsrc) {
  hipPointerAttribute_t at;
  const bool pinned = hipPointerGetAttributes(&at, xyz) == hipSuccess && at.type == hipMemoryTypeHost;
  if (!pinned) (void)hipGetLastError();
  if (pinned) {
    if (stride <= 32) { HIPCHK(c, hipMemcpyAsync(c->staging, xyz, (size_t)(n - 1) * stride + 12, hipMemcpyHostToDevice, s)); }
    else { HIPCHK(c, hipMemcpy2DAsync(c->staging, 16, xyz, stride, 16, n, hipMemcpyHostToDevice, s)); stride = 16; }
    *dsrc = (const char*)c->staging;
    return QN_OK;
  }
  qn_ctx::PinZone& z = c->pin_up;
  if (!z.h) { HIPCHK(c, hipHostMalloc((void**)&z.h, (size_t)c->max_points * 16, hipHostMallocDefault)); HIPCHK(c, hipEventCreateWithFlags(&z.ev, hipEventDisableTiming)); }
  if (z.busy) { HIPCHK(c, hipEventSynchronize(z.ev)); z.busy = false; }
  float* o = (float*)z.h; const char* in = (const char*)xyz;
  for (uint32_t i = 0; i < n; i++, in += stride, o += 3) { const float* p = (const float*)in; o[0] = p[0]; o[1] = p[1]; o[2] = p[2]; }
  HIPCHK(c, hipMemcpyAsync(c->staging, z.h, (size_t)n * 12, hipMemcpyHostToDevice, s));
  HIPCHK(c, hipEventRecord(z.ev, s)); z.busy = true;
  stride = 12; *dsrc = (const char*)c->staging;
  return QN_OK;
}

static int set_cloud(qn_ctx* c, int which, const float* xyz, uint32_t n, uint32_t stride, bool on_device) {
  if (!c || (which != 0 && which != 1)) return QN_ERR_INVALID_ARG;
  CloudBuf& b = c->cloud[which];
  b.n = 0; b.has_grid = b.has_cov = false;
  if (n == 0) return QN_ERR_EMPTY_CLOUD;
  if (!xyz || stride < 12 || (stride & 3)) return QN_ERR_INVALID_ARG;
  if (n > c->max_points) return QN_ERR_CAPACITY;
  HIPCHK(c, hipSetDevice(c->device));
  if (which == QN_SOURCE && join_target(c) != QN_OK) return QN_ERR_HIP;
  c->tgt_on_stream2 = which == QN_TARGET ? (c->pair_pipeline && !c->prof_on && !c->no_pipe && c->cloud[0].has_grid && pair_pipeline_ready(c)) : c->tgt_on_stream2;
  TargetScope scope(c, which == QN_TARGET && c->tgt_on_stream2);
  hipStream_t s = c->stream;
  const char* dsrc = (const char*)xyz;
  if (!on_device) { const int rc = upload_host_cloud(c, xyz, n, stride, s, &dsrc); if (rc != QN_OK) return rc; }
  b.n = n;
  return build_grid(c, b, dsrc, stride);
}

extern "C" int qn_gicp_set_source(qn_ctx* c, const float* xyz, uint32_t n, uint32_t stride) { return set_cloud(c, QN_SOURCE, xyz, n, stride, false); }
extern "C" int qn_gicp_set_target(qn_ctx* c, const float* xyz, uint32_t n, uint32_t stride) { return set_cloud(c, QN_TARGET, xyz, n, stride, false); }
extern "C" int qn_gicp_set_source_device(qn_ctx* c, const float* xyz, uint32_t n, uint32_t stride) { return set_cloud(c, QN_SOURCE, xyz, n, stride, true); }
extern "C" int qn_gicp_set_target_device(qn_ctx* c, const float* xyz, uint32_t n, uint32_t stride) { return set_cloud(c, QN_TARGET, xyz, n, stride, true); }

struct KnnLaunch { KnnHistArgs sel; uint32_t sel_nb; KnnHistArgs lst; uint32_t lst_nb; KnnSingleK::Args single; uint32_t single_nb; KnnCovArgs tail; uint32_t tail_nb; CovFromIdxK::Args cov; uint32_t cov_nb; };
static float knn_first_radius(const qn_ctx* c, const CloudBuf& b) {
  return -(c->margin_knn > 0.f ? c->margin_knn : (b.n > 16384u && b.n <= 65536u ? 2.5f : 2.0f));
}
static KnnLaunch prep_knn(qn_ctx* c, CloudBuf& b, int k, int32_t* kidx, float* kd2, bool lanes = false) {
  const float r0 = knn_first_radius(c, b);
  uint32_t* genc = c->fb_count2 + 1;
  KnnLaunch L;
  L.sel_nb = (b.n + QN_KNN_BLOCK / 4 - 1) / (QN_KNN_BLOCK / 4);
  if (lanes && c->knn_trips > 1) L.sel_nb = (L.sel_nb + (uint32_t)c->knn_trips - 1) / (uint32_t)c->knn_trips;
  L.sel = KnnHistArgs{b.grid, k, r0, c->knn_single_all ? -1 : c->knn_rounds, kidx, kd2, c->fb_list, c->fb_count2, c->big_list, genc};
  L.lst_nb = std::min<uint32_t>((b.n + 63) / 64, lanes ? 96 : 512) * (QN_BLOCK / QN_KNN_BLOCK);
  L.lst = KnnHistArgs{b.grid, k, r0, 64, kidx, kd2, c->fb_list, c->fb_count2, c->big_list, genc};
  L.single_nb = std::min<uint32_t>((b.n + 3) / 4, lanes ? 128 : 2048);
  L.single = KnnSingleK::Args{b.grid, k, kidx, kd2, c->big_list, genc, c->fb_list, c->fb_count2 + 2};
  L.tail_nb = std::min<uint32_t>((b.n + 63) / 64, lanes ? 64 : 1024);
  L.tail = KnnCovArgs{b.grid, b.raw, k, r0, 64, b.nrm, kidx, kd2, c->fb_list, c->fb_count2 + 2};
  L.cov_nb = (b.n + QN_BLOCK - 1) / QN_BLOCK;
  L.cov = CovFromIdxK::Args{b.raw, b.sorted, b.n, k, kidx, b.nrm, &b == &c->cloud[0] ? c->nrm_s_sorted : (double*)nullptr, &b == &c->cloud[0] ? (TargetRec*)nullptr : c->tgt_rec, c->fb_count2};
  return L;
}
template <int KMAX>
static void launch_knn_cov(qn_ctx* c, CloudBuf& b, int k, int32_t* kidx, float* kd2) {
  hipStream_t s = c->stream;
  if (c->knn_hist) {
    const KnnLaunch L = prep_knn(c, b, k, kidx, kd2);
// ... 606 lines not shown
  if (!T || !H || !b6 || !err) return QN_ERR_INVALID_ARG;
  HIPCHK(c, hipSetDevice(c->device));
  hipStream_t s = c->stream;
  HIPCHK(c, hipMemcpyAsync(c->pose_tmp, T, sizeof(double) * 16, hipMemcpyHostToDevice, s));
  hipLaunchKernelGGL(k_set_pose, dim3(1), dim3(64), 0, s, st_cur(c), c->pose_tmp, 0, 0);
  enqueue_nn(c, 0, c->sqd, false); enqueue_accumulate(c, 0, false); enqueue_solve(c, 1, 0);
  GicpState* hs = (GicpState*)malloc(sizeof(GicpState));
  hipError_t e = hipMemcpyAsync(hs, st_cur(c), sizeof(GicpState), hipMemcpyDeviceToHost, s);
  if (e == hipSuccess && corr_out) e = hipMemcpyAsync(corr_out, c->corr, sizeof(int32_t) * c->cloud[0].n, hipMemcpyDeviceToHost, s);
  if (e == hipSuccess && sqd_out) e = hipMemcpyAsync(sqd_out, c->sqd, sizeof(float) * c->cloud[0].n, hipMemcpyDeviceToHost, s);
  if (e == hipSuccess) e = hipStreamSynchronize(s);
  if (e != hipSuccess) { free(hs); c->set_error("linearize readback", e, __LINE__); return QN_ERR_HIP; }
  memcpy(H, hs->H, sizeof(double) * 36); memcpy(b6, hs->b, sizeof(double) * 6); *err = hs->y0;
  free(hs);
  c->prof_collect();
  return clouds_valid(c);
}

extern "C" int qn_gicp_compute_error(qn_ctx* c, const double T[16], double* err) {
  if (c && join_target(c) != QN_OK) return QN_ERR_HIP;
  int rc = ready(c); if (rc != QN_OK) return rc;
  if (!T || !err) return QN_ERR_INVALID_ARG;
  HIPCHK(c, hipSetDevice(c->device));
  hipStream_t s = c->stream;
  HIPCHK(c, hipMemcpyAsync(c->pose_tmp, T, sizeof(double) * 16, hipMemcpyHostToDevice, s));
  hipLaunchKernelGGL(k_set_pose, dim3(1), dim3(64), 0, s, st_cur(c), c->pose_tmp, 1, 1);
  enqueue_accumulate(c, 0, false); enqueue_solve(c, 2, 0);
  HIPCHK(c, hipMemcpyAsync(c->scalar_host, &st_cur(c)->yi, sizeof(double), hipMemcpyDeviceToHost, s));
  HIPCHK(c, hipStreamSynchronize(s));
  *err = c->scalar_host[0];
  c->prof_collect();
  return clouds_valid(c);
}

extern "C" int qn_prof_enable(qn_ctx* c, int on) { if (!c) return QN_ERR_INVALID_ARG; c->prof_on = on != 0; return QN_OK; }
extern "C" int qn_prof_reset(qn_ctx* c) { if (!c) return QN_ERR_INVALID_ARG; c->prof_collect(); for (auto& s : c->stats) { s.total_ms = 0; s.launches = 0; } return QN_OK; }
extern "C" int qn_prof_get(qn_ctx* c, int fam, qn_kernel_stat* out) {
  if (!c || !out || fam < 0 || fam >= QN_K_COUNT) return QN_ERR_INVALID_ARG;
  c->prof_collect(); *out = c->stats[fam]; return QN_OK;
}
extern "C" int qn_debug_set(qn_ctx* c, const char* key, double v) {
  if (!c || !key) return QN_ERR_INVALID_ARG;
  std::string k(key);
  if (k == "cell") { c->cell_override = v; c->cloud[0].has_grid = c->cloud[1].has_grid = false; }
  else if (k == "margin_nn") c->margin_nn = (float)v;
  else if (k == "margin_nn_t0") c->margin_nn_t0 = (float)v;
  else if (k == "big_blocks0") c->big_blocks0 = v < 64 ? 64 : (int)v;
  else if (k == "fb_blocks0") c->fb_blocks0 = v < 64 ? 64 : (int)v;
  else if (k == "margin_knn") c->margin_knn = (float)v;
  else if (k == "knn_single_all") c->knn_single_all = v != 0;
  else if (k == "bbox_blocks") c->bbox_blocks = std::max(1, (int)v);
  else if (k == "device_look") c->device_look = v != 0;
  else if (k == "far_group") c->far_group = (int)v;
  else if (k == "c2f_overlap") c->c2f_overlap = v != 0;
  else if (k == "quatro_fused") c->quatro_fused = v != 0;
  else if (k == "tgt_early") c->tgt_early = v != 0;
  else if (k == "c2f_lanes_fpfh") c->c2f_lanes_fpfh = v != 0;
  else if (k == "normals_fg") c->normals_fg = (int)v;
  else if (k == "fpfh_fg") c->fpfh_fg = (int)v;
  else if (k == "list_small") c->list_small = std::max(0, (int)v);
  else if (k == "far_chunk") c->far_chunk = std::max(1, (int)v);
  else if (k == "far_ranked") c->far_ranked = v != 0;
  else if (k == "batch_look") c->batch_look = v != 0;
  else if (k == "unseeded_cap") c->unseeded_cap = (int)v;
  else if (k == "pair_pipeline") c->pair_pipeline = v != 0;
  else if (k == "persist") c->persist = v != 0;
  else if (k == "persist_timeout") c->persist_timeout = v < 1 ? 1ull : (unsigned long long)v;
  else if (k == "prof_persist") c->prof_persist = v != 0;
  else if (k == "persist_probe") {
    if (v != 0 && !c->pg_clk) { if (hipMalloc(&c->pg_clk, 8 * (64 * 16 + 16)) != hipSuccess) return QN_ERR_HIP; }
    if (c->pg_clk) (void)hipMemset(c->pg_clk, 0, 8 * (64 * 16 + 16));
    if (v == 0) { (void)hipFree(c->pg_clk); c->pg_clk = nullptr; }
  }
  else if (k == "batch_lanes") {
    const int b = std::max(1, std::min((int)v, 64));
    if (b < (int)c->lanes.size()) { if (hipStreamSynchronize(c->stream) != hipSuccess) return QN_ERR_HIP; while ((int)c->lanes.size() > std::max(b, 1)) { qn_ctx* l = c->lanes.back(); c->lanes.pop_back(); if (l != c) qn_ctx_destroy(l); } }
    c->batch_lanes = b; c->lanes_failed = false;
  }
  else if (k == "fail_lane_create") c->fail_lane_create = (int)v;
  else if (k == "batch_share_source") c->batch_share_source = v != 0;
  else if (k == "batch_trace") c->batch_trace = v != 0;
  else if (k == "batch_member") c->persist_batch_off = v != 0;
  else if (k == "stable_cells") c->stable_cells = v != 0;
  else if (k == "knn_hist") c->knn_hist = v != 0;
  else if (k == "nn_rounds") c->nn_rounds = v < 1 ? 1 : (int)v;
  else if (k == "nn_lane") c->nn_lane = v < 0 ? -1 : (v != 0 ? 1 : 0);
  else if (k == "track_from_tick") c->track_from_tick = v < 1 ? 1 : (int)v;
  else if (k == "single_from_tick") c->single_from_tick = v < 1 ? 1 : (int)v;
  else if (k == "fused_from_tick") c->fused_from_tick = v < 1 ? 1 : (int)v;
  else if (k == "knn_rounds") c->knn_rounds = v < 1 ? 1 : (int)v;
  else if (k == "knn_trips") c->knn_trips = v < 1 ? 1 : (int)v;
  else if (k == "knn_mm") c->knn_mm = v != 0;
  else if (k == "fused_ticks") c->fused_ticks = v != 0;
  else if (k == "big_ratio") c->big_ratio = (float)v;
  else if (k == "margin_nn_cap") c->margin_nn_cap = (int)v;
  else if (k == "margin_knn_cap") c->margin_knn_cap = (int)v;
  else if (k == "dbg_counters") {
    if (v != 0 && !c->dbg_counters) { if (hipMalloc(&c->dbg_counters, 16 * sizeof(uint32_t)) != hipSuccess) return QN_ERR_HIP; }
    if (c->dbg_counters) (void)hipMemset(c->dbg_counters, 0, 16 * sizeof(uint32_t));
    if (v == 0) { (void)hipFree(c->dbg_counters); c->dbg_counters = nullptr; }
    for (int w = 0; w < 2; w++) c->cloud[w].grid.dbg = c->dbg_counters;
  }
  else if (k == "ticks_per_chunk") c->ticks_per_chunk = std::max(1, (int)v);
  else if (k == "tick_occ") c->tick_occ = (int)v;
  else if (k == "far") c->far_enabled = v != 0;
  else if (k == "fused_final") c->fused_final = v != 0;
  else if (k == "feat_mfma") c->feat_mfma = v != 0;
  else if (k == "feat_sample") c->feat_sample = (int)v;
  else if (k == "feat_query_dedupe") c->feat_query_dedupe = v != 0;
  else if (k == "feat_min_blocks") c->feat_min_blocks = (int)v;
  else if (k == "feat_verify") { c->feat_verify = v != 0; if (c->q_mm_vcnt) (void)hipMemset(c->q_mm_vcnt, 0, 16); }
  else if (k == "list_probe") {
    if (v != 0 && !c->list_probe) { if (hipMalloc(&c->list_probe, sizeof(unsigned long long) * 4 * 16384) != hipSuccess) return QN_ERR_HIP; }
    if (v == 0 && c->list_probe) { (void)hipFree(c->list_probe); c->list_probe = nullptr; }
  }
  else if (k == "clk_probe") {
    if (v != 0 && !c->clk_probe) { if (hipMalloc(&c->clk_probe, 8 * 8 * 256 + 8 * 12 * 1024) != hipSuccess) return QN_ERR_HIP; }
    if (c->clk_probe) (void)hipMemset(c->clk_probe, 0, 8 * 8 * 256 + 8 * 12 * 1024);
    c->clk_n = 0; if (v == 0) { (void)hipFree(c->clk_probe); c->clk_probe = nullptr; }
  }
  else if (k == "tick_tb") c->tick_tb = v >= 512 ? 512 : 256;
  else if (k == "tick_ppt_min") c->tick_ppt_min = v < 1 ? 1u : (uint32_t)v;
  else if (k == "tick_rpb") c->tick_rpb = v < 1 ? 1u : (uint32_t)v;
  else if (k == "tick_lds_pad") c->tick_lds_pad = v < 0 ? 0 : (int)v;
  else if (k == "knn_lds_pad") c->knn_lds_pad = v < 0 ? 0 : (int)v;
  else if (k == "batch_min_share") c->batch_min_share = v < 1 ? 1 : (int)v;
  else if (k == "verify_track") {
    if (v != 0 && !c->v_counters) {
      const size_t n = c->max_points;
      if (hipMalloc(&c->v_corr, 4 * n) != hipSuccess || hipMalloc(&c->v_nn_idx, 4 * n) != hipSuccess || hipMalloc(&c->v_sqd, 4 * n) != hipSuccess ||
          hipMalloc(&c->v_nn_ref, 16 * n) != hipSuccess || hipMalloc(&c->v_counters, 16) != hipSuccess) return QN_ERR_HIP;
    }
    if (c->v_counters) (void)hipMemset(c->v_counters, 0, 16);
    c->verify_track = v != 0;
  }
  else return QN_ERR_INVALID_ARG;
  return QN_OK;
}
extern "C" int qn_debug_selftest(qn_ctx* c, uint32_t n_waves, uint32_t seed, uint32_t* mismatches) {
  if (!c || !mismatches || n_waves == 0 || n_waves > 65536) return QN_ERR_INVALID_ARG;
  HIPCHK(c, hipSetDevice(c->device));
  std::vector<uint32_t> h((size_t)n_waves * 128);
  uint64_t x = 0x9e3779b97f4a7c15ull ^ seed;
  for (auto& v : h) { x ^= x << 13; x ^= x >> 7; x ^= x << 17; v = (uint32_t)(x >> 16); }
  uint32_t* d = nullptr;
  HIPCHK(c, hipMalloc(&d, (h.size() + 1) * sizeof(uint32_t)));
  int rc = QN_OK; uint32_t bad = 0xffffffffu;
  if (hipMemcpyAsync(d, h.data(), h.size() * sizeof(uint32_t), hipMemcpyHostToDevice, c->stream) != hipSuccess || hipMemsetAsync(d + h.size(), 0, sizeof(uint32_t), c->stream) != hipSuccess) rc = QN_ERR_HIP;
  if (rc == QN_OK) {
    hipLaunchKernelGGL(k_selftest_wave, dim3(n_waves), dim3(64), 0, c->stream, d, d + (size_t)n_waves * 64, d + h.size());
    if (hipMemcpyAsync(&bad, d + h.size(), sizeof(uint32_t), hipMemcpyDeviceToHost, c->stream) != hipSuccess || hipStreamSynchronize(c->stream) != hipSuccess) rc = QN_ERR_HIP;
  }
  (void)hipFree(d);
  if (rc != QN_OK) { c->last_error = "selftest: HIP call failed"; return rc; }
  *mismatches = bad;
  return QN_OK;
}
extern "C" int qn_debug_get_counters(qn_ctx* c, uint32_t out[16]) {
  if (!c || !c->dbg_counters) return QN_ERR_INVALID_ARG;
  if (hipStreamSynchronize(c->stream) != hipSuccess) return QN_ERR_HIP;
  if (hipMemcpy(out, c->dbg_counters, 16 * sizeof(uint32_t), hipMemcpyDeviceToHost) != hipSuccess) return QN_ERR_HIP;
  return QN_OK;
}
extern "C" int qn_debug_get(qn_ctx* c, const char* key, double* value) {
  if (!c || !key || !value) return QN_ERR_INVALID_ARG;
  const std::string k(key);
// ... 63 lines not shown
```

### fast-lio-sam-qn_amd/csrc/qn_gicp_kernels.cuh

```cuda
#pragma once
#include "qn_device.cuh"
#include "qn_knn_hist.cuh"
#include "../../include/qn_engine.h"
#include "qn_util_kernels.cuh"

namespace qn {

#define QN_NPART 28
#define QN_ACC_MAX_BLOCKS 512
#define QN_MAX_TRACE 1024

struct GicpState {
  double x0[16], xi[16], delta[16];
  double H[36], b[6], d[6];
  double y0, yi, den;
  double lambda, nu;
  double final_H[36];
  double fitness;
  int outer, inner, phase, converged, lm_failed;
  uint32_t fb_count;
  uint32_t trace_len;
  uint32_t big_count;
  int pending;
  int reserved;
// ... 157 lines not shown
      uint32_t prefix = 0;
      if (tile == 0) {
        if (lane == 0) __hip_atomic_store(status, tag | (QN_LB_STATE_INC << 32) | agg, __ATOMIC_RELAXED, __HIP_MEMORY_SCOPE_AGENT);
      } else {
        if (lane == 0) __hip_atomic_store(status + tile, tag | (QN_LB_STATE_AGG << 32) | agg, __ATOMIC_RELAXED, __HIP_MEMORY_SCOPE_AGENT);
        int look = (int)tile - 1;
        for (;;) {
          const int mine = look - lane;
          unsigned long long x = 0;
          if (mine >= 0) { do { x = __hip_atomic_load(status + mine, __ATOMIC_RELAXED, __HIP_MEMORY_SCOPE_AGENT); } while ((x >> 34) != (tag >> 34)); }
          const bool is_inc = mine >= 0 && ((x >> 32) & 3ull) == QN_LB_STATE_INC;
          const unsigned long long incs = __ballot(is_inc);
          const int first = incs ? __ffsll((long long)incs) - 1 : 64;
          uint32_t part = (mine >= 0 && lane <= first) ? (uint32_t)x : 0u;
#pragma unroll
          for (int o = 32; o > 0; o >>= 1) part += __shfl_xor(part, o);
          prefix += part;
          if (incs || look - 64 < 0) break;
          look -= 64;
        }
        if (lane == 0) __hip_atomic_store(status + tile, tag | (QN_LB_STATE_INC << 32) | (prefix + agg), __ATOMIC_RELAXED, __HIP_MEMORY_SCOPE_AGENT);
      }
      if (lane == 0) s_prefix = prefix;
    }
    __syncthreads();
    uint32_t run = s_prefix + woff + inc - s;
    if (base + QN_SCAN_ITEMS <= m) {
      uint4* q = (uint4*)(out + base);
#pragma unroll
      for (int j = 0; j < QN_SCAN_ITEMS / 4; j++) { uint4 x; x.x = run; run += v[4 * j]; x.y = run; run += v[4 * j + 1]; x.z = run; run += v[4 * j + 2]; x.w = run; run += v[4 * j + 3]; q[j] = x; }
    } else {
#pragma unroll
      for (int j = 0; j < QN_SCAN_ITEMS; j++) { if (base + j < m) out[base + j] = run; run += v[j]; }
    }
    if (base <= m && m < base + QN_SCAN_ITEMS) out[m] = total;
    if (m == (tile + 1u) * (uint32_t)(QN_BLOCK * QN_SCAN_ITEMS) && threadIdx.x == QN_BLOCK - 1) out[m] = total;
  }
};
static __global__ void __launch_bounds__(QN_BLOCK) k_scan_lookback(const uint32_t* __restrict__ in, const GridDims* __restrict__ dims, uint32_t* __restrict__ out,
                                                                   unsigned long long* status, uint32_t epoch, uint32_t total) {
  const ScanLookbackK::Args a{in, dims, out, status, epoch, total};
  ScanLookbackK::run(a, blockIdx.x, gridDim.x);
}

struct ScatterK {
  static constexpr int TB = QN_BLOCK, OCC = 1;
  struct Args { const float4* pts; uint32_t n; const uint32_t* cell_of_pt; const uint32_t* cell_start; uint32_t* counts; float4* sorted; };
  static __device__ __forceinline__ void run(const Args& a, const uint32_t bx, const uint32_t) {
    const uint32_t i = bx * QN_BLOCK + threadIdx.x;
    if (i >= a.n) return;
    const uint32_t c = a.cell_of_pt[i];
    const uint32_t slot = a.cell_start[c] + atomicSub(&a.counts[c], 1u) - 1u;
    float4 p = a.pts[i];
    p.w = __uint_as_float(i);
    a.sorted[slot] = p;
  }
};
static __global__ void __launch_bounds__(QN_BLOCK) k_scatter(const float4* __restrict__ pts, uint32_t n, const uint32_t* __restrict__ cell_of_pt,
                          const uint32_t* __restrict__ cell_start, uint32_t* __restrict__ counts, float4* __restrict__ sorted) {
  const ScatterK::Args a{pts, n, cell_of_pt, cell_start, counts, sorted};
  ScatterK::run(a, blockIdx.x, gridDim.x);
}

struct StableCellsK {
  static constexpr int TB = QN_BLOCK, OCC = 1;
  struct Args { const float4* in; uint32_t n; const uint32_t* cell_of_pt; const uint32_t* cell_start; float4* out; };
  static __device__ __forceinline__ void run(const Args& a, const uint32_t bx, const uint32_t) {
    const float4* __restrict__ in = a.in; float4* __restrict__ out = a.out;
    const uint32_t t = bx * QN_BLOCK + threadIdx.x;
    if (t >= a.n) return;
    const float4 p = in[t];
    const uint32_t i = __float_as_uint(p.w), c = a.cell_of_pt[i];
    const uint32_t s = a.cell_start[c], e = a.cell_start[c + 1];
    if (e - s > 256u) { out[t] = p; return; }
    uint32_t rank = 0;
    for (uint32_t u = s; u < e; u++) rank += __float_as_uint(in[u].w) < i ? 1u : 0u;
    out[s + rank] = p;
  }
};
static __global__ void __launch_bounds__(QN_BLOCK) k_stable_cells(const float4* __restrict__ in, uint32_t n, const uint32_t* __restrict__ cell_of_pt, const uint32_t* __restrict__ cell_start,
                                      float4* __restrict__ out) {
  const StableCellsK::Args a{in, n, cell_of_pt, cell_start, out};
  StableCellsK::run(a, blockIdx.x, gridDim.x);
}

struct __attribute__((aligned(64))) TargetRec { float4 p; double n[3]; double pad[3]; };
static_assert(sizeof(TargetRec) == 64, "TargetRec is one 64-byte line");
#define QN_COV_BATCH 10
#define QN_COV_REG 20
struct CovFromIdxK {
  static constexpr int TB = QN_BLOCK, OCC = 1;
  struct Args { const float4* raw; const float4* sorted; uint32_t n; int k; const int32_t* knn_idx; double* nrm; double* nrm_sorted; TargetRec* rec; uint32_t* list_counts; };
  static __device__ __forceinline__ void run(const Args& a, const uint32_t bx, const uint32_t nbx) {
    const float4* __restrict__ raw = a.raw; const int32_t* __restrict__ knn_idx = a.knn_idx;
    double* __restrict__ nrm = a.nrm; double* __restrict__ nrm_sorted = a.nrm_sorted; TargetRec* __restrict__ rec = a.rec;
    const int k = a.k;
    if (bx == 0 && threadIdx.x < 4) a.list_counts[threadIdx.x] = 0u;
    const uint32_t spos = xcd_block(bx, nbx) * QN_BLOCK + threadIdx.x;
    if (spos >= a.n) return;
    const uint32_t i = __float_as_uint(a.sorted[spos].w);
    const int32_t* nb = knn_idx + (size_t)i * k;
    int found = 0;
    double mean[3] = {0, 0, 0};
    double nv[3] = {0, 0, 0};
    auto store = [&]() __attribute__((always_inline)) {
#pragma unroll
      for (int u = 0; u < 3; u++) nrm[(size_t)i * 3 + u] = nv[u];
      if (nrm_sorted) {
#pragma unroll
        for (int u = 0; u < 3; u++) nrm_sorted[(size_t)spos * 3 + u] = nv[u];
      }
      if (rec) { TargetRec r; r.p = raw[i];
#pragma unroll
        for (int u = 0; u < 3; u++) { r.n[u] = nv[u]; r.pad[u] = 0; }
        rec[i] = r; }
    };
    double c[6] = {0, 0, 0, 0, 0, 0};
    if (k <= QN_COV_REG) {
      int32_t u[QN_COV_REG]; float4 q[QN_COV_REG];
      static_assert(QN_COV_REG % 4 == 0, "the index row is fetched four entries at a time");
      if ((k & 3) == 0) {
        const int4* __restrict__ nb4 = (const int4*)nb;
#pragma unroll
        for (int e = 0; e < QN_COV_REG; e += 4) {
          const int4 v = e < k ? nb4[e >> 2] : make_int4(-1, -1, -1, -1);
          u[e] = v.x; u[e + 1] = v.y; u[e + 2] = v.z; u[e + 3] = v.w;
        }
      } else {
#pragma unroll
        for (int e = 0; e < QN_COV_REG; e++) u[e] = e < k ? nb[e] : -1;
      }
#pragma unroll
      for (int e = 0; e < QN_COV_REG; e++) q[e] = raw[u[e] < 0 ? 0 : u[e]];
#pragma unroll
      for (int e = 0; e < QN_COV_REG; e++) if (u[e] >= 0) { mean[0] += (double)q[e].x; mean[1] += (double)q[e].y; mean[2] += (double)q[e].z; found++; }
      if (found == 0) { store(); return; }
      mean[0] /= found; mean[1] /= found; mean[2] /= found;
#pragma unroll
      for (int e = 0; e < QN_COV_REG; e++) if (u[e] >= 0) {
        const double dx = (double)q[e].x - mean[0], dy = (double)q[e].y - mean[1], dz = (double)q[e].z - mean[2];
        c[0] += dx * dx; c[1] += dx * dy; c[2] += dx * dz; c[3] += dy * dy; c[4] += dy * dz; c[5] += dz * dz;
      }
    } else {
    for (int j = 0; j < k; j += QN_COV_BATCH) {
      int32_t u[QN_COV_BATCH]; float4 q[QN_COV_BATCH];
#pragma unroll
      for (int e = 0; e < QN_COV_BATCH; e++) u[e] = j + e < k ? nb[j + e] : -1;
#pragma unroll
      for (int e = 0; e < QN_COV_BATCH; e++) q[e] = raw[u[e] < 0 ? 0 : u[e]];
#pragma unroll
      for (int e = 0; e < QN_COV_BATCH; e++) if (u[e] >= 0) { mean[0] += (double)q[e].x; mean[1] += (double)q[e].y; mean[2] += (double)q[e].z; found++; }
    }
    if (found == 0) { store(); return; }
    mean[0] /= found; mean[1] /= found; mean[2] /= found;
    for (int j = 0; j < k; j += QN_COV_BATCH) {
      int32_t u[QN_COV_BATCH]; float4 q[QN_COV_BATCH];
#pragma unroll
      for (int e = 0; e < QN_COV_BATCH; e++) u[e] = j + e < k ? nb[j + e] : -1;
#pragma unroll
      for (int e = 0; e < QN_COV_BATCH; e++) q[e] = raw[u[e] < 0 ? 0 : u[e]];
#pragma unroll
      for (int e = 0; e < QN_COV_BATCH; e++) if (u[e] >= 0) {
        const double dx = (double)q[e].x - mean[0], dy = (double)q[e].y - mean[1], dz = (double)q[e].z - mean[2];
        c[0] += dx * dx; c[1] += dx * dy; c[2] += dx * dz; c[3] += dy * dy; c[4] += dy * dz; c[5] += dz * dz;
      }
    }
// ... 131 lines not shown
  using Args = NnSearchArgs;
  static __device__ __forceinline__ void run(const Args& a, const uint32_t bx, const uint32_t nbx) {
    GridView src = a.src, tgt = a.tgt; const GicpState* __restrict__ st = a.st; const double thr2 = a.thr2; float r0 = a.r0; const int max_rounds = a.max_rounds;
    int32_t* __restrict__ corr = a.corr; float* __restrict__ sqd = a.sqd; int32_t* __restrict__ nn_idx = a.nn_idx; float4* __restrict__ nn_ref = a.nn_ref;
    uint2* __restrict__ fb_list = a.fb_list; uint32_t* __restrict__ fb_count = a.fb_count; uint2* __restrict__ big_list = a.big_list; uint32_t* __restrict__ big_count = a.big_count;
    const int big_blocks = a.big_blocks; const float big_ratio = a.big_ratio; uint32_t* __restrict__ far_stats = a.far_stats; const NnOpt opt = a.opt;

  __shared__ WaveLds lds[BLOCK / 64];
  if (MODE == 0 && uni(st->phase) != 0) return;
  if (MODE == 1 && uni(st->phase) != 2) return;
  if (opt.cond && !(uni(st->reserved) & opt.cond)) return;
  src = grid_resolve(src); tgt = grid_resolve(tgt); if (r0 < 0.f) r0 = -r0 * tgt.cell;
  __shared__ float sTf[12];
  if (threadIdx.x < 12) sTf[threadIdx.x] = (float)st->x0[threadIdx.x];
  __syncthreads();
  if (LIST && (int)bx >= (int)nbx - big_blocks) {
    const uint32_t nbig = uni(*big_count);
    if (tgt.dbg && bx == nbx - 1 && threadIdx.x == 0) atomicAdd(&tgt.dbg[7], nbig);
    uint32_t nfar = 0;
    const uint32_t bw0 = (bx - (nbx - big_blocks)) * (BLOCK / 64) + (threadIdx.x >> 6), nbw = big_blocks * (BLOCK / 64);
    const uint32_t E = (GROUP && opt.group && nbig >= (uint32_t)opt.group_min) ? min(16u, (nbig + (uint32_t)opt.group - 1u) / (uint32_t)opt.group) : 1u;
    if (GROUP && E > 1u) {
      const int lane = threadIdx.x & 63, qs = lane & 15;
      WaveLds* wl = &lds[threadIdx.x >> 6];
      const float INF = __int_as_float(0x7f800000);
      for (uint32_t w0 = bw0 * E; w0 < nbig; w0 += nbw * E) {
        const uint32_t slot = w0 + (uint32_t)qs;
        const bool active = (uint32_t)qs < E && slot < nbig;
        const uint2 rec = active ? big_list[slot] : make_uint2(0u, 0u);
        const float4 p = active ? src.pts[rec.x] : make_float4(0.f, 0.f, 0.f, 0.f);
        float qx, qy, qz; { float Tf[12];
#pragma unroll
          for (int j = 0; j < 12; j++) Tf[j] = sTf[j];
          xform_query<MODE>(Tf, p.x, p.y, p.z, qx, qy, qz); }
        const float v = __uint_as_float(rec.y);
        const float r = v > 0.f ? v * 1.1f + 0.5f * tgt.cell : -v;
        const bool finite_q = (qx - qx == 0.f) && (qy - qy == 0.f) && (qz - qz == 0.f) && (r - r == 0.f);
        unsigned long long key = QN_INF_KEY; float second = INF, d_unseen = INF;
        unsigned long long todo = __ballot(active);
        while (todo) {
          const int al = __ffsll((long long)todo) - 1;
          const float ax = rdlane(qx, al), ay = rdlane(qy, al), az = rdlane(qz, al), ar = rdlane(r, al);
          const bool afin = rdlane((int)finite_q, al) != 0;
          const bool open_q = (todo >> lane) & 1ull;
          const bool member = open_q && (qs == (al & 15) || (afin && finite_q && sqdist(qx, qy, qz, ax, ay, az) <= 0.25f * ar * ar));
          const unsigned long long mm = __ballot(member);
          if (__popcll(mm) <= 4) {
            unsigned long long k1; float s1, du1;
            wave_search_single(tgt, ax, ay, az, ar, INF, k1, s1, du1, wl);
            if (member) { key = k1; second = s1; d_unseen = du1; }
          } else {
            wave_search_far16(tgt, qx, qy, qz, member, r, key, second, d_unseen, wl);
          }
          todo &= ~mm;
        }
        if (active && lane < 16) {
          const uint32_t tl = late(rec.x);
          store_nn<MODE>(key, late(__float_as_uint(p.w)), tl, thr2, corr, sqd, nn_idx);
          if (MODE == 0) nn_ref[tl] = make_float4(qx, qy, qz, key != QN_INF_KEY ? sqrtf(key_d2(key)) : INF);
        }
        if (far_stats && MODE == 0) {
          const unsigned long long fm = __ballot(active && lane < 16 && key != QN_INF_KEY && key_d2(key) > 36.f * tgt.cell * tgt.cell);
          if (lane == 0) nfar += (uint32_t)__popcll(fm);
        }
      }
      if (far_stats && MODE == 0 && (threadIdx.x & 63) == 0 && nfar) atomicAdd(&far_stats[3], nfar);
      return;
    }
    unsigned long long pr_sum = 0, pr_max = 0, pr_a = 0, pr_b = 0; uint32_t pr_n = 0;
    const uint32_t nfb_all = uni(*fb_count);
    const uint32_t nfb1 = (opt.fb_small && nfb_all <= opt.fb_small) ? nfb_all : 0u;
    for (uint32_t w = bw0; w < nbig + nfb1; w += nbw) {
      const uint2 rec = w < nbig ? big_list[w] : fb_list[w - nbig];
      const float4 p = src.pts[rec.x];
      float qx, qy, qz; { float Tf[12];
#pragma unroll
          for (int j = 0; j < 12; j++) Tf[j] = sTf[j];
          xform_query<MODE>(Tf, p.x, p.y, p.z, qx, qy, qz); }
      const float v = __uint_as_float(rec.y);
      const float r = v > 0.f ? v * 1.1f + 0.5f * tgt.cell : -v;
      unsigned long long key; float second, d_unseen;
      const unsigned long long pt0 = opt.probe ? wall_clock64() : 0ull;
      SingleStats sst;
      wave_search_single(tgt, qx, qy, qz, r, __int_as_float(0x7f800000), key, second, d_unseen, &lds[threadIdx.x >> 6], sst, opt.probe != nullptr);
      if (opt.probe) { const unsigned long long dt = wall_clock64() - pt0; pr_sum += dt; pr_n++;
        if (dt > pr_max) { pr_max = dt; pr_a = ((unsigned long long)sst.rounds << 48) | ((unsigned long long)min(sst.segs, 0xffffffu) << 24) | (unsigned long long)min(sst.cand, 0xffffffu);
          pr_b = ((unsigned long long)__float_as_uint(sst.r_first) << 32) | __float_as_uint(key != QN_INF_KEY ? sqrtf(key_d2(key)) : -1.f); } }
      if ((threadIdx.x & 63) == 0) {
        const uint32_t tl = late(rec.x);
        store_nn<MODE>(key, late(__float_as_uint(p.w)), tl, thr2, corr, sqd, nn_idx);
        if (MODE == 0) nn_ref[tl] = make_float4(qx, qy, qz, fminf(sqrtf(second), d_unseen));
        if (key != QN_INF_KEY && key_d2(key) > 36.f * tgt.cell * tgt.cell) nfar++;
      }
    }
    if (far_stats && MODE == 0 && (threadIdx.x & 63) == 0 && nfar) atomicAdd(&far_stats[3], nfar);
    if (opt.probe && (threadIdx.x & 63) == 0 && bw0 < 16384u) { opt.probe[4 * bw0] = (pr_max << 32) | pr_n; opt.probe[4 * bw0 + 1] = pr_sum; opt.probe[4 * bw0 + 2] = pr_a; opt.probe[4 * bw0 + 3] = pr_b; }
    return;
  }
  const uint32_t nq = LIST ? uni(*fb_count) : src.n;
  if (LIST && opt.fb_small && nq <= opt.fb_small) return;
  if (LIST && tgt.dbg && bx == 0 && threadIdx.x == 0) atomicAdd(&tgt.dbg[5], nq);
  const uint32_t wave0 = bx * (BLOCK / 64) + (threadIdx.x >> 6), nwaves = (nbx - (LIST ? big_blocks : 0)) * (BLOCK / 64);
  for (uint32_t base = wave0 * 16; base < nq; base += nwaves * 16) {
    const uint32_t slot = base + (threadIdx.x & 15);
    const bool active = slot < nq;
    uint32_t t = slot; float r = r0, r_cap = __int_as_float(0x7f800000);
    if (LIST && active) {
      const uint2 rec = fb_list[slot]; t = rec.x;
      const float v = __uint_as_float(rec.y);
      if (v < 0.f) r = -v; else { r_cap = v; r = fminf(v, r0); }
    }
    const float4 p = active ? src.pts[t] : make_float4(0, 0, 0, 0);
    float qx, qy, qz; { float Tf[12];
#pragma unroll
          for (int j = 0; j < 12; j++) Tf[j] = sTf[j];
          xform_query<MODE>(Tf, p.x, p.y, p.z, qx, qy, qz); }
    Best1 sink; sink.init();
    float d_unseen;
    const bool cert = wave_search<4>(tgt, qx, qy, qz, active, r, r_cap, max_rounds, sink, &lds[threadIdx.x >> 6], d_unseen);
    const bool mine = active && (threadIdx.x & 48) == 0;
    const bool done = cert || LIST;
    if (!LIST && MODE == 0 && opt.clear_ref && mine) opt.clear_ref[t] = make_float4(0.f, 0.f, 0.f, 0.f);
    if (mine && done) {
      const uint32_t tl = late(t);
      store_nn<MODE>(sink.key, late(__float_as_uint(p.w)), tl, thr2, corr, sqd, nn_idx);
      if (MODE == 0) nn_ref[tl] = make_float4(qx, qy, qz, fminf(sqrtf(sink.second), d_unseen));
    }
    if (!LIST) {
      const float rn = r;
      const bool far = rn > big_ratio * r0;
      wave_append(big_list, big_count, mine && !done && far, make_uint2(t, __float_as_uint(-rn)));
      wave_append(fb_list, fb_count, mine && !done && !far, make_uint2(t, __float_as_uint(-rn)));
    }
  }
  }
};
template <int MODE, bool LIST, int BLOCK, bool GROUP = false>
__global__ void __launch_bounds__(BLOCK, GROUP ? 5 : 6) k_nn_search(GridView src, GridView tgt, const GicpState* __restrict__ st, double thr2, float r0, int max_rounds,
                                                        int32_t* __restrict__ corr, float* __restrict__ sqd, int32_t* __restrict__ nn_idx, float4* __restrict__ nn_ref,
                                                        uint2* __restrict__ fb_list, uint32_t* __restrict__ fb_count,
                                                        uint2* __restrict__ big_list, uint32_t* __restrict__ big_count, int big_blocks, float big_ratio, uint32_t* __restrict__ far_stats, NnOpt opt) {
  const NnSearchArgs a{src, tgt, st, thr2, r0, max_rounds, corr, sqd, nn_idx, nn_ref, fb_list, fb_count, big_list, big_count, big_blocks, big_ratio, far_stats, opt};
  NnSearchK<MODE, LIST, BLOCK, GROUP>::run(a, blockIdx.x, gridDim.x);
}

__device__ __forceinline__ void accumulate_point_n(const double (*Rx)[4], const double (*Tx)[4], const float4 pa, const float4 pb,
                                                   const double na[3], const double nb[3], const bool lin, double acc[QN_NPART]) {
  double m[3];
#pragma unroll
  for (int a = 0; a < 3; a++) m[a] = Rx[a][0] * na[0] + Rx[a][1] * na[1] + Rx[a][2] * na[2];
  M3 rcr;
#pragma unroll
  for (int a = 0; a < 3; a++)
#pragma unroll
    for (int b = a; b < 3; b++) {
      const double g = Rx[a][0] * Rx[b][0] + Rx[a][1] * Rx[b][1] + Rx[a][2] * Rx[b][2];
      rcr.m[a][b] = ((a == b ? 1.0 : 0.0) - 0.999 * nb[a] * nb[b]) + (g - 0.999 * m[a] * m[b]);
      rcr.m[b][a] = rcr.m[a][b];
    }
  const M3 M = m3_inverse(rcr);
  const double mA[3] = {(double)pa.x, (double)pa.y, (double)pa.z};
  double tA[3], e[3], Me[3];
#pragma unroll
  for (int r = 0; r < 3; r++) tA[r] = Tx[r][0] * mA[0] + Tx[r][1] * mA[1] + Tx[r][2] * mA[2] + Tx[r][3];
  e[0] = (double)pb.x - tA[0]; e[1] = (double)pb.y - tA[1]; e[2] = (double)pb.z - tA[2];
#pragma unroll
  for (int r = 0; r < 3; r++) Me[r] = M.m[r][0] * e[0] + M.m[r][1] * e[1] + M.m[r][2] * e[2];
// ... 678 lines not shown
```

### fast-lio-sam-qn_amd/csrc/qn_tick.cuh

```cuda
#pragma once
#include "qn_gicp_kernels.cuh"

namespace qn {


struct TickArgs {
  GridView src, tgt;
  TailArgs tail;
  double* part_out;
  double thr2;
  int32_t* nn_idx; float4* nn_ref;
  const double* nrm_s;
  const TargetRec* tgt_rec;
  uint32_t ppt;
  uint32_t rpb, rows;
  int far_mode;
  const float4* tgt_raw;
  int32_t* cand; float4* cand_ref;
  float2* cand_b;
  unsigned long long* far_req;
  uint32_t* far_stats;
  float4* aligned; double* fit_psum; uint32_t* fit_pcnt;
  unsigned long long* clk;
  unsigned long long* clk_blk;
// ... 536 lines not shown
  double* far_rows;
  uint32_t ranked_max;
  uint32_t* far_stats;
};
struct FarK {
  static constexpr int TB = QN_FAR_THREADS, OCC = 1;
  using Args = FarArgs;
  static __device__ __forceinline__ void run(const FarArgs& a_in, const uint32_t bx, const uint32_t) {
    FarArgs a = a_in;

  __shared__ WaveLdsH1 lds[QN_FAR_THREADS / 64];
  __shared__ double wsum[QN_FAR_THREADS / 64][QN_NPART];
  __shared__ uint32_t wpre[QN_FAR_WORDS];
  __shared__ uint32_t wtot[QN_FAR_THREADS / 64];
  const int tid = threadIdx.x, lane = tid & 63, wid = tid >> 6;
  constexpr int NW = QN_FAR_THREADS / 64;
  a.src = grid_resolve(a.src); a.tgt = grid_resolve(a.tgt);
  const int phase = uni(a.st->phase);
  double acc[QN_NPART];
#pragma unroll
  for (int u = 0; u < QN_NPART; u++) acc[u] = 0;
  if (phase == 0 && uni(a.st->pending)) {
    float Tf[12]; double X0[3][4];
#pragma unroll
    for (int j = 0; j < 12; j++) Tf[j] = uni((float)a.st->x0[j]);
#pragma unroll
    for (int r = 0; r < 3; r++)
#pragma unroll
      for (int c = 0; c < 4; c++) X0[r][c] = uni(a.st->x0[4 * r + c]);
    const uint32_t nchunks = (a.src.n + 63u) >> 6;
    const bool ranked = nchunks <= min((uint32_t)QN_FAR_WORDS, a.ranked_max);
    uint32_t total_req = 0;
    if (ranked && uni(a.far_stats[0]) != 0u) {
      for (uint32_t w = tid; w < nchunks; w += QN_FAR_THREADS) wpre[w] = (uint32_t)__popcll(a.far_req[w]);
      __syncthreads();
      constexpr uint32_t PER = (QN_FAR_WORDS + QN_FAR_THREADS - 1) / QN_FAR_THREADS;
      uint32_t loc[PER], sum = 0;
#pragma unroll
      for (uint32_t u = 0; u < PER; u++) { const uint32_t w = tid * PER + u; loc[u] = w < nchunks ? wpre[w] : 0u; sum += loc[u]; }
      uint32_t inc = wave_incl_scan_u32(sum, lane);
      if (lane == 63) wtot[wid] = inc;
      __syncthreads();
      uint32_t base = inc - sum;
      for (int w2 = 0; w2 < wid; w2++) base += wtot[w2];
      for (int w2 = 0; w2 < NW; w2++) total_req += wtot[w2];
      __syncthreads();
#pragma unroll
      for (uint32_t u = 0; u < PER; u++) { const uint32_t w = tid * PER + u; if (w < nchunks) wpre[w] = base; base += loc[u]; }
      __syncthreads();
    }
    const uint32_t gw = bx * NW + wid, ngw = QN_FAR_BLOCKS * NW;
    uint32_t seen = 0;
    uint32_t e = gw;
    uint32_t ch = ranked ? 0u : bx;
    unsigned long long word = 0;
    for (;;) {
      uint32_t t;
      if (ranked) {
        if (e >= total_req) break;
        uint32_t lo = 0;
        for (uint32_t step = 1u << 11; step > 0; step >>= 1) { const uint32_t w = lo + step; if (w < nchunks && wpre[w] <= e) lo = w; }
        unsigned long long wd = a.far_req[lo];
        for (uint32_t skip = e - wpre[lo]; skip > 0; skip--) wd &= wd - 1;
        t = lo * 64u + (uint32_t)(__ffsll((long long)wd) - 1);
        e += ngw;
      } else {
        while (word == 0) { if (ch >= nchunks) break; word = a.far_req[ch]; if (word == 0) ch += QN_FAR_BLOCKS; }
        if (word == 0) break;
        t = ch * 64u + (uint32_t)(__ffsll((long long)word) - 1);
        word &= word - 1; if (word == 0) ch += QN_FAR_BLOCKS;
        const bool mine_req = (int)(seen % NW) == wid; seen++;
        if (!mine_req) continue;
      }
      {
        const float4 p = a.src.pts[t];
        float qx, qy, qz; xform_query<0>(Tf, p.x, p.y, p.z, qx, qy, qz);
        const uint32_t j0 = (uint32_t)a.nn_idx[t];
        float r = 2.f * a.tgt.cell;
        if (j0 < a.tgt.n) { const float4 p0 = a.tgt_raw[j0]; r = sqrtf(sqdist(qx, qy, qz, p0.x, p0.y, p0.z)) * 1.002f + 0.4f * a.tgt.cell; }
        int32_t* cl = a.cand + (size_t)t * QN_FAR_M;
        unsigned long long best = QN_INF_KEY; float second = __int_as_float(0x7f800000), bound = 0.f, other = __int_as_float(0x7f800000), b4 = 0.f, b16 = 0.f;
        float dnn = -1.f;
        if (j0 < a.tgt.n) { const float4 p0 = a.tgt_raw[j0]; dnn = sqrtf(sqdist(qx, qy, qz, p0.x, p0.y, p0.z)); }
        else { float du; wave_search_single(a.tgt, qx, qy, qz, r, __int_as_float(0x7f800000), best, second, du, &lds[wid].s); if (best != QN_INF_KEY) dnn = sqrtf(key_d2(best)); other = fminf(sqrtf(second), du); }
        if (dnn >= 0.f) {
          const float4 lastq = a.nn_ref[t];
          const float moved = sqrtf(sqdist(qx, qy, qz, lastq.x, lastq.y, lastq.z));
          float m = fminf(fmaxf(fmaxf(2.f * a.tgt.cell * a.tgt.cell / fmaxf(dnn, a.tgt.cell), 2.5f * moved), 0.01f), 0.5f * a.tgt.cell);
          for (int attempt = 0; attempt < 5; attempt++, m *= 0.5f) {
            const float R = dnn * 1.000002f + a.tgt.eps + m;
            const uint32_t cnt = wave_ball_collect(a.tgt, qx, qy, qz, R, &lds[wid].s, lds[wid].list, &lds[wid].cnt, best, second);
            other = fminf(sqrtf(second), R * 0.9999995f);
            if (cnt <= (uint32_t)QN_FAR_M && cnt > 0) {
              const unsigned long long own = (uint32_t)lane < cnt ? lds[wid].list[lane] : QN_INF_KEY;
              int rank = 0;
              for (uint32_t f = 0; f < cnt; f++) rank += lds[wid].list[f] < own ? 1 : 0;
              if ((uint32_t)lane < cnt) cl[rank] = (int32_t)key_idx(own); else if (lane < QN_FAR_M) cl[lane] = -1;
              bound = R * 0.9999995f;
              const unsigned long long k5 = wave_min_u64(rank == 4 && own != QN_INF_KEY ? own : QN_INF_KEY), k17 = wave_min_u64(rank == 16 && own != QN_INF_KEY ? own : QN_INF_KEY);
              b4 = k5 != QN_INF_KEY ? fminf(sqrtf(key_d2(k5)) * 0.9999995f, bound) : bound;
              b16 = k17 != QN_INF_KEY ? fminf(sqrtf(key_d2(k17)) * 0.9999995f, bound) : bound;
              break;
            }
          }
        }
        if (lane == 0) {
          a.nn_idx[t] = best != QN_INF_KEY ? (int32_t)key_idx(best) : -1;
          a.nn_ref[t] = make_float4(qx, qy, qz, other);
          a.cand_ref[t] = make_float4(qx, qy, qz, bound); a.cand_b[t] = make_float2(b4, b16);
          if (best != QN_INF_KEY && (double)key_d2(best) < a.thr2) {
            const TargetRec* rec = a.tgt_rec + key_idx(best);
            const double na[3] = {a.nrm_s[(size_t)t * 3], a.nrm_s[(size_t)t * 3 + 1], a.nrm_s[(size_t)t * 3 + 2]};
            const double nb[3] = {rec->n[0], rec->n[1], rec->n[2]};
            accumulate_point_n(X0, X0, make_float4(p.x, p.y, p.z, 1.f), rec->p, na, nb, true, acc);
          }
        }
      }
    }
  }
  if (lane == 0) {
#pragma unroll
    for (int u = 0; u < QN_NPART; u++) wsum[wid][u] = acc[u];
  }
  __syncthreads();
  if (tid < QN_NPART) { double v = 0;
#pragma unroll
    for (int w = 0; w < NW; w++) v += wsum[w][tid]; a.far_rows[(size_t)bx * QN_NPART + tid] = v; }
  }
};
static __global__ void __launch_bounds__(QN_FAR_THREADS) k_far(FarArgs a) { FarK::run(a, blockIdx.x, gridDim.x); }
struct FarReduceK {
  static constexpr int TB = QN_FAR_BLOCKS, OCC = 1;
  struct Args { const double* far_rows; double* part; int rows; uint32_t* far_stats; TailArgs tail; };
  static __device__ __forceinline__ void run(const Args& a, const uint32_t, const uint32_t) {
    __shared__ double sh[QN_FAR_BLOCKS / 32][QN_NPART];
    __shared__ TailLds tl;
    const double* __restrict__ far_rows = a.far_rows; double* part_row = a.part + (size_t)a.rows * QN_NPART; uint32_t* __restrict__ far_stats = a.far_stats;
    const int tid = threadIdx.x, c = tid % 32, seg = tid / 32;
    if (tid == 0) { far_stats[1] = far_stats[0]; far_stats[0] = 0u; }
    if (c < QN_NPART) {
      double v[32];
#pragma unroll
      for (int u = 0; u < 32; u++) v[u] = far_rows[(size_t)(seg * 32 + u) * QN_NPART + c];
      double acc = 0;
#pragma unroll
      for (int u = 0; u < 32; u++) acc += v[u];
      sh[seg][c] = acc;
    }
    __syncthreads();
    if (tid < QN_NPART) { double v = 0; for (int s2 = 0; s2 < QN_FAR_BLOCKS / 32; s2++) v += sh[s2][tid]; row_store(&part_row[tid], v, true); }
    if (!a.tail.enabled) return;
    asm volatile("s_waitcnt vmcnt(0)" ::: "memory");
    __syncthreads();
    for (int i = tid; i < (int)(sizeof(GicpState) / 8); i += TB) ((unsigned long long*)&tl.sh)[i] = ((const unsigned long long*)a.tail.st_in)[i];
    reduce_rows<TB, true>(a.part, a.rows + 1, tl.part, tl.sums);
    if (tid == 0) {
      const int phase = tl.sh.phase;
      if (tl.sh.pending && phase != 2) { const GicpConfig cfg = a.tail.cfg; solve_controller(&tl.sh, tl.sums, cfg, a.tail.trace, 0, phase, &tl.work); }
      tl.sh.fb_count = 0; tl.sh.big_count = 0; tl.sh.pending = tl.sh.phase != 2 ? 1 : 0;
    }
    __syncthreads();
    for (int i = tid; i < (int)(sizeof(GicpState) / 8); i += TB) ((unsigned long long*)a.tail.st_out)[i] = ((const unsigned long long*)&tl.sh)[i];
  }
};
static __global__ void __launch_bounds__(QN_FAR_BLOCKS) k_far_reduce(FarReduceK::Args a) { FarReduceK::run(a, blockIdx.x, gridDim.x); }

}
// ... 1 lines not shown
```

Measured before the change: 4409.

## Prune target grid tiles and rows with tight point bounding boxes

Adds a kernel that computes, for the target cloud, tight axis-aligned bounding boxes of the points actually stored in each 128-cell tile and each 8-cell row segment. The neighbour search and ball-collect routines use these boxes to drop tiles or rows whose real contents lie outside the search radius, and use the nearest skipped box distance to grow the radius less aggressively. The aim is to cut wasted candidate scans over sparsely occupied cells. The cost is an extra grid-build kernel, extra memory for the boxes, and more per-segment arithmetic in the search loops. Some callers strip the boxes to keep their previous behaviour.

```diff
diff --git a/fast-lio-sam-qn_amd/csrc/qn_batch.inc b/fast-lio-sam-qn_amd/csrc/qn_batch.inc
--- a/fast-lio-sam-qn_amd/csrc/qn_batch.inc
+++ b/fast-lio-sam-qn_amd/csrc/qn_batch.inc
@@ -104,7 +104,7 @@
     if (l->params.k_correspondences != c->params.k_correspondences) l->cloud[0].has_cov = l->cloud[1].has_cov = false;
     l->params = c->params;
     l->cell_override = c->cell_override; l->margin_nn = c->margin_nn; l->margin_nn_t0 = c->margin_nn_t0; l->margin_knn = c->margin_knn; l->big_blocks0 = c->big_blocks0; l->fb_blocks0 = c->fb_blocks0;
-    l->big_ratio = c->big_ratio; l->nn_rounds = c->nn_rounds; l->knn_rounds = c->knn_rounds; l->knn_trips = c->knn_trips; l->knn_mm = c->knn_mm; l->knn_single_all = c->knn_single_all; l->bbox_blocks = c->bbox_blocks; l->stable_cells = c->stable_cells;
+    l->big_ratio = c->big_ratio; l->nn_rounds = c->nn_rounds; l->knn_rounds = c->knn_rounds; l->knn_trips = c->knn_trips; l->knn_mm = c->knn_mm; l->knn_single_all = c->knn_single_all; l->bbox_blocks = c->bbox_blocks; l->stable_cells = c->stable_cells; l->tight_bounds = c->tight_bounds;
     l->unseeded_cap = c->unseeded_cap; l->track_from_tick = c->track_from_tick; l->fused_from_tick = c->fused_from_tick; l->ticks_per_chunk = c->ticks_per_chunk; l->far_chunk = c->far_chunk; l->far_group = c->far_group; l->far_ranked = c->far_ranked;
     l->list_small = c->list_small; l->tick_ppt_min = c->tick_ppt_min; l->tick_rpb = c->tick_rpb; l->nn_lane = c->nn_lane;
   }
@@ -127,11 +127,12 @@
   } alias_guard(L, last_src);
   struct FailGuard { std::vector<LaneRun>& L; int* status; bool armed = true; ~FailGuard() { if (armed) for (const LaneRun& R : L) if (R.active) status[R.pair] = QN_ERR_HIP; } } fail_guard{L, status};
   std::vector<LaneEntry<PackBBoxK::Args>> v_pack; std::vector<LaneEntry<CellCountK::Args>> v_count; std::vector<LaneEntry<ScanLookbackK::Args>> v_scan;
-  std::vector<LaneEntry<ScatterK::Args>> v_scat; std::vector<LaneEntry<StableCellsK::Args>> v_stab;
+  std::vector<LaneEntry<ScatterK::Args>> v_scat; std::vector<LaneEntry<StableCellsK::Args>> v_stab; std::vector<LaneEntry<TightBoundsK::Args>> v_tight;
   std::vector<LaneEntry<KnnHistArgs>> v_sel, v_lst; std::vector<LaneEntry<KnnSingleK::Args>> v_single; std::vector<LaneEntry<KnnCovArgs>> v_tail; std::vector<LaneEntry<CovFromIdxK::Args>> v_cov;
   auto push_grid = [&](const GridLaunch& G) {
     lane_push(v_pack, G.pack, G.pack_nb); lane_push(v_count, G.count, G.nb); lane_push(v_scan, G.scan, G.scan_nb); lane_push(v_scat, G.scat, G.nb);
     if (G.stable) lane_push(v_stab, G.stab, G.nb);
+    if (G.tight_on) lane_push(v_tight, G.tight, G.tight_nb);
   };
   auto push_knn = [&](const KnnLaunch& K) {
     lane_push(v_sel, K.sel, K.sel_nb); lane_push(v_lst, K.lst, K.lst_nb); lane_push(v_single, K.single, K.single_nb); lane_push(v_tail, K.tail, K.tail_nb); lane_push(v_cov, K.cov, K.cov_nb);
@@ -168,7 +169,7 @@
     last_src[l] = R.alias >= 0 ? nullptr : pd.src; last_key[l] = key;
     R.active = true;
   }
-  plan.add<PackBBoxK>(v_pack, QN_K_GRID_BUILD); plan.add<CellCountK>(v_count, QN_K_GRID_BUILD); plan.add<ScanLookbackK>(v_scan, QN_K_GRID_BUILD); plan.add<ScatterK>(v_scat, QN_K_GRID_BUILD); plan.add<StableCellsK>(v_stab, QN_K_GRID_BUILD);
+  plan.add<PackBBoxK>(v_pack, QN_K_GRID_BUILD); plan.add<CellCountK>(v_count, QN_K_GRID_BUILD); plan.add<ScanLookbackK>(v_scan, QN_K_GRID_BUILD); plan.add<ScatterK>(v_scat, QN_K_GRID_BUILD); plan.add<StableCellsK>(v_stab, QN_K_GRID_BUILD); plan.add<TightBoundsK>(v_tight, QN_K_GRID_BUILD);
   if (k <= 24) { if (owner->knn_mm) plan.add<KnnHistK<false, 32>>(v_sel, QN_K_KNN_SELECT, (uint32_t)owner->knn_lds_pad); else plan.add<KnnHistK<false, 32, false>>(v_sel, QN_K_KNN_SELECT, (uint32_t)owner->knn_lds_pad); plan.add<KnnHistK<true, 32>>(v_lst, QN_K_KNN_COV); } else { plan.add<KnnHistK<false, 48>>(v_sel, QN_K_KNN_SELECT); plan.add<KnnHistK<true, 48>>(v_lst, QN_K_KNN_COV); }
   plan.add<KnnSingleK>(v_single, QN_K_KNN_COV);
   if (k <= 16) plan.add<KnnCovK<16, true, 4>>(v_tail, QN_K_KNN_COV); else if (k <= 20) plan.add<KnnCovK<20, true, 4>>(v_tail, QN_K_KNN_COV); else if (k <= 24) plan.add<KnnCovK<24, true, 4>>(v_tail, QN_K_KNN_COV); else plan.add<KnnCovK<32, true, 4>>(v_tail, QN_K_KNN_COV);
diff --git a/fast-lio-sam-qn_amd/csrc/qn_context.h b/fast-lio-sam-qn_amd/csrc/qn_context.h
--- a/fast-lio-sam-qn_amd/csrc/qn_context.h
+++ b/fast-lio-sam-qn_amd/csrc/qn_context.h
@@ -14,6 +14,8 @@
   uint32_t* cell_start = nullptr;
   uint32_t* counts = nullptr;
   double* nrm = nullptr;
+  float4* tbox = nullptr;
+  float4* rbox = nullptr;
   qn::GridView grid{};
   qn::GridDims* dims = nullptr;
   qn::GridDims* dims_host = nullptr;
@@ -91,7 +93,7 @@
   int big_blocks0 = 4096, fb_blocks0 = 512;
   float margin_nn_t0 = 0.f;
   float margin_nn = 1.f, margin_knn = 0.f;
-  int margin_nn_cap = 3, margin_knn_cap = 5, ticks_per_chunk = 8; bool knn_single_all = false, stable_cells = true; int bbox_blocks = 64;
+  int margin_nn_cap = 3, margin_knn_cap = 5, ticks_per_chunk = 8; bool knn_single_all = false, stable_cells = true, tight_bounds = true; int bbox_blocks = 64;
   hipStream_t stream2 = nullptr; hipEvent_t ev_pair = nullptr; bool pair_pipeline = true, pair_failed = false, tgt_on_stream2 = false, tgt_pending = false, no_pipe = false;
   uint32_t* scan_sums2 = nullptr; uint2* fb_list2 = nullptr; uint2* big_list2 = nullptr; uint32_t* fb_count2b = nullptr; int32_t* knn_idx2 = nullptr;
   uint32_t tick_ppt_min = 1;
diff --git a/fast-lio-sam-qn_amd/csrc/qn_device.cuh b/fast-lio-sam-qn_amd/csrc/qn_device.cuh
--- a/fast-lio-sam-qn_amd/csrc/qn_device.cuh
+++ b/fast-lio-sam-qn_amd/csrc/qn_device.cuh
@@ -19,6 +19,8 @@
   const float4* pts;
   const uint32_t* cell_start;
   uint32_t* dbg;
+  const float4* tbox;
+  const float4* rbox;
   float ox, oy, oz, cell, inv_cell, eps;
   int nx, ny, nz;
   int ntx, nty, ntz;
@@ -351,6 +353,12 @@
   const float yl = g.oy + (float)(ty << 2) * g.cell, yh = g.oy + (float)min((ty << 2) + 4, g.ny) * g.cell;
   const float zl = g.oz + (float)(tz << 2) * g.cell, zh = g.oz + (float)min((tz << 2) + 4, g.nz) * g.cell;
   const float dx = fmaxf(fmaxf(xl - qx, qx - xh) - g.eps, 0.f), dy = fmaxf(fmaxf(yl - qy, qy - yh) - g.eps, 0.f), dz = fmaxf(fmaxf(zl - qz, qz - zh) - g.eps, 0.f);
+  return ((dx * dx + dy * dy) + dz * dz) * 0.999998f;
+}
+
+__device__ __forceinline__ float tight_box_d2(const float4* __restrict__ box, uint32_t i, float qx, float qy, float qz) {
+  const float4 lo = box[2 * i], hi = box[2 * i + 1];
+  const float dx = fmaxf(fmaxf(lo.x - qx, qx - hi.x), 0.f), dy = fmaxf(fmaxf(lo.y - qy, qy - hi.y), 0.f), dz = fmaxf(fmaxf(lo.z - qz, qz - hi.z), 0.f);
   return ((dx * dx + dy * dy) + dz * dz) * 0.999998f;
 }
 
@@ -378,7 +386,10 @@
         int qz_, ry_; divmod_small(r, ntyr, qz_, ry_);
         const int tzz = (z0 >> 2) + qz_, tyy = ty0 + ry_, txx = tx0 + t;
         const uint32_t tile = ((uint32_t)tzz * g.nty + tyy) * g.ntx + txx;
-        if (!(ball_r2 >= 0.f && tile_box_d2(g, txx, tyy, tzz, bqx, bqy, bqz) > ball_r2)) { s = g.cell_start[tile << 7]; len = g.cell_start[(tile + 1) << 7] - s; }
+        if (!(ball_r2 >= 0.f && tile_box_d2(g, txx, tyy, tzz, bqx, bqy, bqz) > ball_r2)) {
+          s = g.cell_start[tile << 7]; len = g.cell_start[(tile + 1) << 7] - s;
+          if (ball_r2 >= 0.f && g.tbox && tight_box_d2(g.tbox, tile, bqx, bqy, bqz) > ball_r2) len = 0;
+        }
       } else {
         int qz_, ry_; divmod_small(r, nyr, qz_, ry_);
         const int ry = y0 + ry_, rz = z0 + qz_, tx = tx0 + t;
@@ -625,6 +636,7 @@
     const int nyr = y1 - y0 + 1;
     if (!tile_mode || done2 < 0.f) { best = QN_INF_KEY; second = INF; done2 = -1.f; }
     const float in2 = r * r * 1.000002f;
+    float skip2 = INF;
     for (int sb = 0; sb < nseg; sb += 64) {
       const int sidx = sb + lane;
       uint32_t s = 0, len = 0;
@@ -635,14 +647,28 @@
           const int tzz = (z0 >> 2) + qz_, tyy = ty0 + ry_, txx = tx0 + t;
           const uint32_t tile = ((uint32_t)tzz * g.nty + tyy) * g.ntx + txx;
           const float tb2 = tile_box_d2(g, txx, tyy, tzz, qx, qy, qz);
-          const bool seen = tb2 <= done2 && txx >= ptx0 && txx <= ptx1 && tyy >= pty0 && tyy <= pty1 && tzz >= ptz0 && tzz <= ptz1;
-          if (!(tb2 > in2) && !seen) { s = g.cell_start[tile << 7]; len = g.cell_start[(tile + 1) << 7] - s; }
+          if (g.tbox) {
+            if (!(tb2 > in2)) {
+              s = g.cell_start[tile << 7]; len = g.cell_start[(tile + 1) << 7] - s;
+              const float m2 = fmaxf(tb2, tight_box_d2(g.tbox, tile, qx, qy, qz));
+              const bool seen = m2 <= done2 && txx >= ptx0 && txx <= ptx1 && tyy >= pty0 && tyy <= pty1 && tzz >= ptz0 && tzz <= ptz1;
+              if (m2 > in2 && len) skip2 = fminf(skip2, m2);
+              if (m2 > in2 || seen) len = 0;
+            }
+          } else {
+            const bool seen = tb2 <= done2 && txx >= ptx0 && txx <= ptx1 && tyy >= pty0 && tyy <= pty1 && tzz >= ptz0 && tzz <= ptz1;
+            if (!(tb2 > in2) && !seen) { s = g.cell_start[tile << 7]; len = g.cell_start[(tile + 1) << 7] - s; }
+          }
         } else {
           int qz_, ry_; divmod_small(rr, nyr, qz_, ry_);
           const int ry = y0 + ry_, rz = z0 + qz_, tx = tx0 + t;
           const int xa = max(x0, tx << 3), xb = min(x1, (tx << 3) + 7);
           const uint32_t k0 = cell_key(g, xa, ry, rz);
           s = g.cell_start[k0]; len = g.cell_start[k0 + (xb - xa) + 1] - s;
+          if (g.rbox && len) {
+            const float m2 = tight_box_d2(g.rbox, k0 >> 3, qx, qy, qz);
+            if (m2 > in2) { skip2 = fminf(skip2, m2); len = 0; }
+          }
         }
       }
       const uint32_t incl = wave_incl_scan_u32(len, lane);
@@ -680,11 +706,13 @@
     if (z0 > 0) d = fminf(d, cap_face_dist(cap, qz - (g.oz + z0 * g.cell), 2));
     if (z1 < g.nz - 1) d = fminf(d, cap_face_dist(cap, (g.oz + (z1 + 1) * g.cell) - qz, 2));
     bool cert;
-    if (tile_mode && r == r && round <= 160) d = fminf(d, r * 0.999998f + g.eps);
+    const float sk2 = (g.tbox || g.rbox) ? wave_min_f(skip2) : INF;
+    if ((tile_mode || sk2 < INF) && r == r && round <= 160) d = fminf(d, r * 0.999998f + g.eps);
     if (d == INF || !(r == r) || round > 160) { cert = true; d_unseen = INF; }
     else { d -= g.eps; d_unseen = d; cert = d > 0.f && b != QN_INF_KEY && key_d2(b) < d * d; }
     if (cert) { best_out = b; second_out = c; return; }
     r = (b != QN_INF_KEY) ? fmaxf(sqrtf(key_d2(b)) * 1.000001f + g.eps, r + g.eps) : (r > 6.f * g.cell ? r + (2.f + round) * g.cell : 2.f * r + g.cell);
+    if (b == QN_INF_KEY && sk2 < INF) r = fminf(r, fmaxf(sqrtf(sk2) * 1.000001f + g.eps, r + g.eps));
     r = fminf(r, r_cap);
   }
 }
@@ -735,6 +763,7 @@
     const int nseg = ntr * ntyr * ((z1 >> 2) - tz0 + 1);
     const float in2 = R * R * 1.000002f;
     bool left_out = false;
+    float skip2 = INF;
     for (int sb = 0; sb < nseg; sb += 64) {
       const int sidx = sb + lane;
       uint32_t s = 0, len = 0;
@@ -744,9 +773,17 @@
         const int tzz = tz0 + qz_, tyy = ty0 + ry_, txx = tx0 + t;
         const uint32_t tile = ((uint32_t)tzz * g.nty + tyy) * g.ntx + txx;
         const float tb2 = tile_box_d2(g, txx, tyy, tzz, cqx, cqy, cqz);
-        const bool seen = tb2 <= done2 && txx >= ptx0 && txx <= ptx1 && tyy >= pty0 && tyy <= pty1 && tzz >= ptz0 && tzz <= ptz1;
         if (tb2 > in2) left_out = true;
-        else if (!seen) { s = g.cell_start[tile << 7]; len = g.cell_start[(tile + 1) << 7] - s; }
+        else if (g.tbox) {
+          s = g.cell_start[tile << 7]; len = g.cell_start[(tile + 1) << 7] - s;
+          const float m2 = fmaxf(tb2, tight_box_d2(g.tbox, tile, cqx, cqy, cqz));
+          const bool seen = m2 <= done2 && txx >= ptx0 && txx <= ptx1 && tyy >= pty0 && tyy <= pty1 && tzz >= ptz0 && tzz <= ptz1;
+          if (m2 > in2 && len) { left_out = true; skip2 = fminf(skip2, m2); }
+          if (m2 > in2 || seen) len = 0;
+        } else {
+          const bool seen = tb2 <= done2 && txx >= ptx0 && txx <= ptx1 && tyy >= pty0 && tyy <= pty1 && tzz >= ptz0 && tzz <= ptz1;
+          if (!seen) { s = g.cell_start[tile << 7]; len = g.cell_start[(tile + 1) << 7] - s; }
+        }
       }
       const uint32_t incl = wave_incl_scan_u32(len, lane);
       const uint32_t total = rdlane(incl, 63);
@@ -790,7 +827,11 @@
     }
     if (!__any(open)) break;
     const float want = wave_max_f(need);
-    const float grown = want > 0.f ? want : (R > 6.f * g.cell ? R + (2.f + round) * g.cell : 2.f * R + g.cell);
+    float grown = want > 0.f ? want : (R > 6.f * g.cell ? R + (2.f + round) * g.cell : 2.f * R + g.cell);
+    if (g.tbox && !(want > 0.f)) {
+      const float sk2 = wave_min_f(skip2);
+      if (sk2 < INF) grown = fminf(grown, sqrtf(sk2) * 1.000002f + g.eps);
+    }
     R = fmaxf(grown, R * 1.0001f + g.eps);
   }
   const unsigned long long ob = __shfl(fin_b, my_rank & 63); const float os = __shfl(fin_s, my_rank & 63), od = __shfl(fin_d, my_rank & 63);
diff --git a/fast-lio-sam-qn_amd/csrc/qn_engine.hip b/fast-lio-sam-qn_amd/csrc/qn_engine.hip
--- a/fast-lio-sam-qn_amd/csrc/qn_engine.hip
+++ b/fast-lio-sam-qn_amd/csrc/qn_engine.hip
@@ -86,6 +86,10 @@
   sl.take(b.counts, sizeof(uint32_t) * ((size_t)c->max_cells + 1));
   sl.take(b.nrm, sizeof(double) * 3 * c->max_points);
   sl.take(b.dims, sizeof(GridDims));
+  if (&b == &c->cloud[1]) {
+    sl.take(b.tbox, sizeof(float4) * 2 * (c->max_cells / QN_TILE_CELLS));
+    sl.take(b.rbox, sizeof(float4) * 2 * (c->max_cells / 8));
+  }
 }
 
 static int ctx_create(int device, uint32_t max_points, hipStream_t shared_stream, qn_ctx** out);
@@ -270,7 +274,8 @@
   return hipStreamWaitEvent(c->stream, c->ev_pair, 0) == hipSuccess ? QN_OK : QN_ERR_HIP;
 }
 
-struct GridLaunch { PackBBoxK::Args pack; uint32_t pack_nb; CellCountK::Args count; ScanLookbackK::Args scan; uint32_t scan_nb; ScatterK::Args scat; StableCellsK::Args stab; bool stable; uint32_t nb; };
+struct GridLaunch { PackBBoxK::Args pack; uint32_t pack_nb; CellCountK::Args count; ScanLookbackK::Args scan; uint32_t scan_nb; ScatterK::Args scat; StableCellsK::Args stab; bool stable; uint32_t nb;
+                    TightBoundsK::Args tight; uint32_t tight_nb; bool tight_on; };
 static GridLaunch prep_grid(qn_ctx* c, CloudBuf& b, const char* dsrc, uint32_t stride, bool lanes = false) {
   const uint32_t n = b.n;
   GridView& g = b.grid;
@@ -287,6 +292,10 @@
   L.stable = c->stable_cells;
   L.scat = ScatterK::Args{b.raw, n, b.cell_of_pt, b.cell_start, b.counts, L.stable ? b.sorted_tmp : b.sorted};
   L.stab = StableCellsK::Args{b.sorted_tmp, n, b.cell_of_pt, b.cell_start, b.sorted};
+  L.tight_on = c->tight_bounds && b.tbox && b.rbox;
+  L.tight = TightBoundsK::Args{b.sorted, b.cell_start, b.dims, b.tbox, b.rbox};
+  L.tight_nb = (c->max_cells / QN_TILE_CELLS + QN_BLOCK / 64 - 1) / (QN_BLOCK / 64);
+  if (L.tight_on) { g.tbox = b.tbox; g.rbox = b.rbox; }
   b.has_grid = true; b.has_cov = false;
   return L;
 }
@@ -298,7 +307,8 @@
     hipLaunchKernelGGL(k_cell_count, dim3(L.nb), dim3(QN_BLOCK), 0, s, L.count.pts, L.count.n, L.count.g, L.count.counts, L.count.cell_of_pt);
     hipLaunchKernelGGL(k_scan_lookback, dim3(L.scan_nb), dim3(QN_BLOCK), 0, s, L.scan.in, L.scan.dims, L.scan.out, L.scan.status, L.scan.epoch, L.scan.total);
     hipLaunchKernelGGL(k_scatter, dim3(L.nb), dim3(QN_BLOCK), 0, s, L.scat.pts, L.scat.n, L.scat.cell_of_pt, L.scat.cell_start, L.scat.counts, L.scat.sorted);
-    if (L.stable) hipLaunchKernelGGL(k_stable_cells, dim3(L.nb), dim3(QN_BLOCK), 0, s, L.stab.in, L.stab.n, L.stab.cell_of_pt, L.stab.cell_start, L.stab.out); }
+    if (L.stable) hipLaunchKernelGGL(k_stable_cells, dim3(L.nb), dim3(QN_BLOCK), 0, s, L.stab.in, L.stab.n, L.stab.cell_of_pt, L.stab.cell_start, L.stab.out);
+    if (L.tight_on) hipLaunchKernelGGL(k_tight_bounds, dim3(L.tight_nb), dim3(QN_BLOCK), 0, s, L.tight.pts, L.tight.cell_start, L.tight.dims, L.tight.tbox, L.tight.rbox); }
   HIPCHK(c, hipGetLastError());
   return QN_OK;
 }
@@ -1071,6 +1081,7 @@
   else if (k == "batch_trace") c->batch_trace = v != 0;
   else if (k == "batch_member") c->persist_batch_off = v != 0;
   else if (k == "stable_cells") c->stable_cells = v != 0;
+  else if (k == "tight_bounds") { if (c->tight_bounds != (v != 0)) { c->tight_bounds = v != 0; c->cloud[1].has_grid = false; } }
   else if (k == "knn_hist") c->knn_hist = v != 0;
   else if (k == "nn_rounds") c->nn_rounds = v < 1 ? 1 : (int)v;
   else if (k == "nn_lane") c->nn_lane = v < 0 ? -1 : (v != 0 ? 1 : 0);
diff --git a/fast-lio-sam-qn_amd/csrc/qn_gicp_kernels.cuh b/fast-lio-sam-qn_amd/csrc/qn_gicp_kernels.cuh
--- a/fast-lio-sam-qn_amd/csrc/qn_gicp_kernels.cuh
+++ b/fast-lio-sam-qn_amd/csrc/qn_gicp_kernels.cuh
@@ -263,6 +263,42 @@
                                       float4* __restrict__ out) {
   const StableCellsK::Args a{in, n, cell_of_pt, cell_start, out};
   StableCellsK::run(a, blockIdx.x, gridDim.x);
+}
+
+struct TightBoundsK {
+  static constexpr int TB = QN_BLOCK, OCC = 1;
+  struct Args { const float4* pts; const uint32_t* cell_start; const GridDims* dims; float4* tbox; float4* rbox; };
+  static __device__ __forceinline__ void run(const Args& a, const uint32_t bx, const uint32_t) {
+    const uint32_t tile = bx * (QN_BLOCK / 64) + (threadIdx.x >> 6);
+    const uint32_t ntiles = uni(a.dims->ncells) >> 7;
+    if (tile >= ntiles) return;
+    const int lane = threadIdx.x & 63;
+    const uint32_t row = (tile << 4) | (uint32_t)(lane & 15);
+    const uint32_t s = a.cell_start[row << 3], e = a.cell_start[(row << 3) + 8];
+    const float INF = __int_as_float(0x7f800000);
+    float lx = INF, ly = INF, lz = INF, hx = -INF, hy = -INF, hz = -INF;
+    for (uint32_t u = s + (uint32_t)(lane >> 4); u < e; u += 4u) {
+      const float4 p = a.pts[u];
+      lx = fminf(lx, p.x); ly = fminf(ly, p.y); lz = fminf(lz, p.z); hx = fmaxf(hx, p.x); hy = fmaxf(hy, p.y); hz = fmaxf(hz, p.z);
+    }
+#pragma unroll
+    for (int o = 16; o < 64; o <<= 1) {
+      lx = fminf(lx, __shfl_xor(lx, o)); ly = fminf(ly, __shfl_xor(ly, o)); lz = fminf(lz, __shfl_xor(lz, o));
+      hx = fmaxf(hx, __shfl_xor(hx, o)); hy = fmaxf(hy, __shfl_xor(hy, o)); hz = fmaxf(hz, __shfl_xor(hz, o));
+    }
+    if (lane < 16 && e > s) { a.rbox[2 * row] = make_float4(lx, ly, lz, 0.f); a.rbox[2 * row + 1] = make_float4(hx, hy, hz, 0.f); }
+#pragma unroll
+    for (int o = 1; o < 16; o <<= 1) {
+      lx = fminf(lx, __shfl_xor(lx, o)); ly = fminf(ly, __shfl_xor(ly, o)); lz = fminf(lz, __shfl_xor(lz, o));
+      hx = fmaxf(hx, __shfl_xor(hx, o)); hy = fmaxf(hy, __shfl_xor(hy, o)); hz = fmaxf(hz, __shfl_xor(hz, o));
+    }
+    if (lane == 0) { a.tbox[2 * tile] = make_float4(lx, ly, lz, 0.f); a.tbox[2 * tile + 1] = make_float4(hx, hy, hz, 0.f); }
+  }
+};
+static __global__ void __launch_bounds__(QN_BLOCK) k_tight_bounds(const float4* __restrict__ pts, const uint32_t* __restrict__ cell_start, const GridDims* __restrict__ dims,
+                                                                  float4* __restrict__ tbox, float4* __restrict__ rbox) {
+  const TightBoundsK::Args a{pts, cell_start, dims, tbox, rbox};
+  TightBoundsK::run(a, blockIdx.x, gridDim.x);
 }
 
 struct __attribute__((aligned(64))) TargetRec { float4 p; double n[3]; double pad[3]; };
@@ -560,7 +596,8 @@
       unsigned long long key; float second, d_unseen;
       const unsigned long long pt0 = opt.probe ? wall_clock64() : 0ull;
       SingleStats sst;
-      wave_search_single(tgt, qx, qy, qz, r, __int_as_float(0x7f800000), key, second, d_unseen, &lds[threadIdx.x >> 6], sst, opt.probe != nullptr);
+      GridView tgt_cell = tgt; tgt_cell.tbox = nullptr; tgt_cell.rbox = nullptr;
+      wave_search_single(tgt_cell, qx, qy, qz, r, __int_as_float(0x7f800000), key, second, d_unseen, &lds[threadIdx.x >> 6], sst, opt.probe != nullptr);
       if (opt.probe) { const unsigned long long dt = wall_clock64() - pt0; pr_sum += dt; pr_n++;
         if (dt > pr_max) { pr_max = dt; pr_a = ((unsigned long long)sst.rounds << 48) | ((unsigned long long)min(sst.segs, 0xffffffu) << 24) | (unsigned long long)min(sst.cand, 0xffffffu);
           pr_b = ((unsigned long long)__float_as_uint(sst.r_first) << 32) | __float_as_uint(key != QN_INF_KEY ? sqrtf(key_d2(key)) : -1.f); } }
diff --git a/fast-lio-sam-qn_amd/csrc/qn_tick.cuh b/fast-lio-sam-qn_amd/csrc/qn_tick.cuh
--- a/fast-lio-sam-qn_amd/csrc/qn_tick.cuh
+++ b/fast-lio-sam-qn_amd/csrc/qn_tick.cuh
@@ -642,7 +642,8 @@
         unsigned long long best = QN_INF_KEY; float second = __int_as_float(0x7f800000), bound = 0.f, other = __int_as_float(0x7f800000), b4 = 0.f, b16 = 0.f;
         float dnn = -1.f;
         if (j0 < a.tgt.n) { const float4 p0 = a.tgt_raw[j0]; dnn = sqrtf(sqdist(qx, qy, qz, p0.x, p0.y, p0.z)); }
-        else { float du; wave_search_single(a.tgt, qx, qy, qz, r, __int_as_float(0x7f800000), best, second, du, &lds[wid].s); if (best != QN_INF_KEY) dnn = sqrtf(key_d2(best)); other = fminf(sqrtf(second), du); }
+        else { float du; GridView tg = a.tgt; tg.tbox = nullptr; tg.rbox = nullptr;
+          wave_search_single(tg, qx, qy, qz, r, __int_as_float(0x7f800000), best, second, du, &lds[wid].s); if (best != QN_INF_KEY) dnn = sqrtf(key_d2(best)); other = fminf(sqrtf(second), du); }
         if (dnn >= 0.f) {
           const float4 lastq = a.nn_ref[t];
           const float moved = sqrtf(sqdist(qx, qy, qz, lastq.x, lastq.y, lastq.z));
```

After: 4426, median of 6. No clear change (+0.4%).
